# fevzibabaoglu/adaptive-edge-aware-jpeg

Measured on AMD Instinct MI355X. Metric: megapixels/sec encode (Canny+quadtree+DCT+quant), 4K batch, higher is better.
Workload: dtype f32; 1 GPU; 64 x 3840x2160 float32 RGB per GPU, YCbCr, blocks 4-64, quality 40-80 (BASELINE config 4: 512 4K images / 8 GPUs); images_per_gpu=64, height=2160, width=3840, color_space=YCbCr, steps_in_flight=4

## Files before the change

### adaptive_edge_aware_jpeg_amd/_lib.py

```python
import ctypes
import os
import threading

import numpy as np

_HERE = os.path.dirname(os.path.abspath(__file__))
LIB_PATH = os.environ.get("AEJ_LIBRARY") or os.path.join(_HERE, "libaejpeg_hip.so")

SPACE_IDS = {"YCbCr": 0, "YCoCg": 1, "YCoCg-R": 2, "OKLAB": 3, "ICtCp": 4, "ICaCb": 5, "JzAzBz": 6}
CONVERT_IDS = dict(SPACE_IDS, XYZ=7)

AEJ_ERR_ARG, AEJ_ERR_HIP, AEJ_ERR_STATE, AEJ_ERR_CAPACITY, AEJ_ERR_UNSUPPORTED = -1, -2, -3, -4, -5


class AejError(RuntimeError):
    pass


class AejPlan(ctypes.Structure):
    _fields_ = [
        ("batch", ctypes.c_int32), ("H", ctypes.c_int32), ("W", ctypes.c_int32),
        ("layer_h", ctypes.c_int32 * 3), ("layer_w", ctypes.c_int32 * 3), ("root_size", ctypes.c_int32 * 3),
        ("coeff_off", ctypes.c_int64 * 3), ("coeff_stride", ctypes.c_int64),
        ("leaf_off", ctypes.c_int64 * 3), ("leaf_stride", ctypes.c_int64),
        ("state_off", ctypes.c_int64 * 3), ("state_stride", ctypes.c_int64),
        ("workspace_bytes", ctypes.c_uint64),
    ]


_lib = None
_lib_lock = threading.Lock()

HIP_DEFAULT_HW_QUEUES = 4
_hw_queues = HIP_DEFAULT_HW_QUEUES
_hw_queues_source = "HIP default (assumed)"


def _look_at_hw_queues():
    global _hw_queues, _hw_queues_source
    present = os.environ.get("GPU_MAX_HW_QUEUES")
    if present is not None:
        try:
            v = int(present)
        except ValueError:
            v = 0
        if v > 0:
            _hw_queues, _hw_queues_source = v, "GPU_MAX_HW_QUEUES was in the environment when the package was imported"
    return _hw_queues


def configure_hw_queues(want=16):
    global _hw_queues, _hw_queues_source
    import sys
    if os.environ.get("GPU_MAX_HW_QUEUES") is not None:
        return _look_at_hw_queues()
    trusted = "torch" not in sys.modules
    os.environ["GPU_MAX_HW_QUEUES"] = str(int(want))
    if trusted:
        _hw_queues, _hw_queues_source = int(want), "configure_hw_queues() before torch was imported"
        for ctx in _contexts.values():
            ctx.check(ctx.lib.aej_set_hw_queues(ctx.handle, _hw_queues))
    return _hw_queues


def set_hw_queues(n):
    global _hw_queues, _hw_queues_source
    _hw_queues, _hw_queues_source = int(n), "stated by the application (set_hw_queues)"
    for ctx in _contexts.values():
        ctx.check(ctx.lib.aej_set_hw_queues(ctx.handle, _hw_queues))


def hw_queues():
    return _hw_queues, _hw_queues_source


_warned_queue_limited = False


def warn_if_queue_limited(ctx, batch, H, W):
    global _warned_queue_limited
    if _warned_queue_limited:
        return
    sch = ctx.schedule(batch, H, W)
    if sch["limited_by_hw_queues"]:
        _warned_queue_limited = True
        import warnings
        warnings.warn(f"adaptive_edge_aware_jpeg_amd: this call ({batch} x {W}x{H}) would run as more overlapping sub-batches with more hardware "
                      f"queues; the library schedules for {sch['hw_queues']} ({_hw_queues_source}).  Put GPU_MAX_HW_QUEUES=16 into the environment "
                      "(or call adaptive_edge_aware_jpeg_amd.configure_hw_queues()) before `import torch`, or state the runtime's real value with "
                      "set_hw_queues().", RuntimeWarning, stacklevel=3)


_P, _I, _I64, _U64 = ctypes.c_void_p, ctypes.c_int, ctypes.c_int64, ctypes.c_uint64
class CannyParams(ctypes.Structure):
    _fields_ = [("canny_low_ratio", ctypes.c_double), ("canny_high_ratio", ctypes.c_double), ("clahe_clip_limit", ctypes.c_double),
                ("bilateral_sigma_color", ctypes.c_double), ("bilateral_sigma_space", ctypes.c_double), ("use_l2_gradient", ctypes.c_int)]


class JpegDecHuff(ctypes.Structure):
    _fields_ = [("lut", ctypes.c_uint16 * 512), ("maxcode", ctypes.c_int32 * 18), ("valoff", ctypes.c_int32 * 18), ("vals", ctypes.c_uint8 * 256)]


class JpegDecDesc(ctypes.Structure):
    _fields_ = [("width", ctypes.c_int32), ("height", ctypes.c_int32), ("ncomp", ctypes.c_int32), ("hs", ctypes.c_int32), ("vs", ctypes.c_int32),
                ("mcux", ctypes.c_int32), ("mcuy", ctypes.c_int32), ("blocks_per_mcu", ctypes.c_int32), ("restart_interval", ctypes.c_int32),
                ("n_segments", ctypes.c_int32), ("sof", ctypes.c_int32), ("precision16", ctypes.c_int32),
                ("comp_id", ctypes.c_uint8 * 4), ("comp_h", ctypes.c_uint8 * 4), ("comp_v", ctypes.c_uint8 * 4), ("comp_tq", ctypes.c_uint8 * 4),
                ("qt", (ctypes.c_uint16 * 64) * 3), ("dc", JpegDecHuff * 3), ("ac", JpegDecHuff * 3),
                ("scan_offset", ctypes.c_int64), ("scan_length", ctypes.c_int64)]


class JpegProgFrame(ctypes.Structure):
    _fields_ = [("width", ctypes.c_int32), ("height", ctypes.c_int32), ("ncomp", ctypes.c_int32), ("hs", ctypes.c_int32), ("vs", ctypes.c_int32),
                ("mcux", ctypes.c_int32), ("mcuy", ctypes.c_int32), ("blocks_per_mcu", ctypes.c_int32), ("sof", ctypes.c_int32),
                ("precision16", ctypes.c_int32), ("n_scans", ctypes.c_int32), ("n_levels", ctypes.c_int32),
                ("comp_id", ctypes.c_uint8 * 4), ("comp_h", ctypes.c_uint8 * 4), ("comp_v", ctypes.c_uint8 * 4), ("comp_tq", ctypes.c_uint8 * 4),
                ("qt", (ctypes.c_uint16 * 64) * 3)]


class JpegProgScan(ctypes.Structure):
    _fields_ = [("ncomp", ctypes.c_int32), ("comp", ctypes.c_int32 * 4), ("td", ctypes.c_int32 * 4), ("ta", ctypes.c_int32 * 4),
                ("ss", ctypes.c_int32), ("se", ctypes.c_int32), ("ah", ctypes.c_int32), ("al", ctypes.c_int32),
                ("restart_interval", ctypes.c_int32), ("units_x", ctypes.c_int32), ("units_y", ctypes.c_int32),
                ("n_segments", ctypes.c_int32), ("level", ctypes.c_int32), ("dc", JpegDecHuff * 3), ("ac", JpegDecHuff),
                ("data_offset", ctypes.c_int64), ("data_length", ctypes.c_int64)]


SIGNATURES = {
    "aej_abi_version": (_I, []),
    "aej_create": (_P, [_I, _P]),
    "aej_destroy": (None, [_P]),
    "aej_last_error": (ctypes.c_char_p, [_P]),
    "aej_synchronize": (_I, [_P]),
    "aej_set_stream": (_I, [_P, _P]),
    "aej_get_hysteresis_stats": (_I, [_P, _P]),
    "aej_set_graph_mode": (_I, [_P, _I]),
    "aej_set_sub_batches": (_I, [_P, _I]),
    "aej_set_hw_queues": (_I, [_P, _I]),
    "aej_get_schedule_host": (_I, [_P, _I, _I, _I, _P]),
    "aej_set_option": (_I, [_P, ctypes.c_char_p, _I64]),
    "aej_get_option": (_I, [_P, ctypes.c_char_p, _P]),
    "aej_test_fail_after_stage": (_I, [_P, _I]),
    "aej_encode_batch_begin": (_I, [_P, _P, _I, _I, _I, _I, _P, _P, _P, _P, _P, _P, _U64]),
    "aej_encode_batch_end": (_I, [_P]),
    "aej_get_split_calls": (ctypes.c_int64, [_P]),
    "aej_get_graph_stats": (_I, [_P, _P]),
    "aej_set_profiling": (_I, [_P, _I]),
    "aej_get_stage_ms": (_I, [_P, _P]),
    "aej_stage_name": (ctypes.c_char_p, [_I]),
    "aej_set_settings": (_I, [_P, _I, _I, _I, _P]),
    "aej_encode_plan": (_I, [_P, _I, _I, _I, ctypes.POINTER(AejPlan)]),
    "aej_encode_batch": (_I, [_P, _P, _I, _I, _I, _P, _P, _P, _P, _P, _P, _U64]),
    "aej_encode_batch_u8": (_I, [_P, _P, _I, _I, _I, _P, _P, _P, _P, _P, _P, _U64]),
    "aej_metrics_workspace_bytes": (_U64, [_I, _I, _I]),
    "aej_metrics_batch": (_I, [_P, _P, _P, _I, _I, _I, _I, _P, _P, _U64]),
    "aej_color_convert": (_I, [_P, _I, _P, _P, _I64]),
    "aej_color_planes": (_I, [_P, _P, _I, _I, _I, _P, _P, _P]),
    "aej_canny_workspace_bytes": (_U64, [_I, _I]),
    "aej_canny": (_I, [_P, _P, _I, _I, _P, _P, _P, _P, _U64]),
    "aej_set_canny_params": (_I, [_P, _P]),
    "aej_quadtree_workspace_bytes": (_U64, [_I, _I, _I, _I]),
    "aej_quadtree_capacity": (_I, [_I, _I, _I, _I, ctypes.POINTER(_I64), ctypes.POINTER(_I64), ctypes.POINTER(_I64)]),
    "aej_quadtree": (_I, [_P, _P, _I, _I, _I, _I, _P, _P, _P, _P, _U64]),
    "aej_dct_quant_zigzag": (_I, [_P, _P, _I, _I, _I, _P, _I64, _P, _P]),
    "aej_deflate_stream_bound": (_U64, [_U64]),
    "aej_deflate_workspace_bytes": (_U64, [_P, _I, _I, _I]),
    "aej_deflate_histogram": (_I, [_P, _P, _P, _I, _I, _I, _P, _P, _U64]),
    "aej_deflate_batch": (_I, [_P, _P, _P, _I, _I, _I, _P, _I, _P, _U64, _P, _P, _U64]),
    "aej_deflate_build_tables": (_I, [_P, _P, _P]),
    "aej_pack_u8_levels_host": (_I, [_P, _I64, _P, _I]),
    "aej_decode_workspace_bytes": (_U64, [_P, _I, _I, _I]),
    "aej_decode_batch": (_I, [_P, _P, _P, _P, _I, _I, _I, _P, _P, _U64]),
    "aej_decode_batch_tables": (_I, [_P, _P, _P, _P, _I, _I, _I, _P, _P, _P, _U64]),
    "aej_requantise_batch": (_I, [_P, _P, _P, _P, _I, _I, _I, _I, _P, _P, _U64]),
    "aej_color_convert_inverse": (_I, [_P, _I, _P, _P, _I64]),
    "aej_leaf_positions_host": (_I64, [_P, _I64, _I, _I, _I, _P]),
    "aej_inflate_batch": (_I, [_P, _P, _P, _I, _P, _U64, _P, _P]),
    "aej_decode_headers_workspace_bytes": (_U64, [_P, _I, _I, _I]),
    "aej_decode_headers": (_I, [_P, _P, _P, _P, _I, _I, _I, _P, _P, _P, _P, _U64]),
    "aej_lpips_weights_bytes": (_U64, []),
    "aej_lpips_param_count": (_I64, []),
    "aej_lpips_pack_weights_host": (_I, [_P, _I64, _P]),
    "aej_lpips_features_bytes": (_U64, [_I, _I, _I]),
    "aej_lpips_workspace_bytes": (_U64, [_I, _I, _I]),
    "aej_lpips_features": (_I, [_P, _P, _P, _I, _I, _I, _P, _P, _U64]),
    "aej_lpips_batch": (_I, [_P, _P, _P, _P, _P, _I, _I, _I, _P, _P, _U64]),
    "aej_jfif_workspace_bytes": (_U64, [_I, _I, _I, _I]),
    "aej_jfif_headers_host": (_I, [_I, _I, _I, _P, _I]),
    "aej_jfif_encode_batch": (_I, [_P, _P, _I, _I, _I, _I, _P, _P, _U64, _P, _P, _P, _P, _U64]),
    "aej_jfif_recon_batch": (_I, [_P, _I, _I, _I, _I, _P, _P, _U64]),
    "aej_jfif_workspace_bytes_opt": (_U64, [_I, _I, _I, _I, _I, _I]),
    "aej_jfif_headers_host_opt": (_I, [_I, _I, _I, _I, _P, _I]),
    "aej_jfif_huffman_host": (_I, [_P, _P, _P, _I]),
    "aej_jfif_encode_batch_opt": (_I, [_P, _P, _I, _I, _I, _I, _P, _I, _I, _P, _U64, _P, _P, _P, _P, _U64]),
    "aej_jfif_recon_batch_opt": (_I, [_P, _I, _I, _I, _I, _I, _I, _P, _P, _U64]),
    "aej_jpegdec_parse_host": (_I, [_P, _U64, _P, _P, _I]),
    "aej_jpegdec_workspace_bytes": (_U64, [_P, _P, _I]),
    "aej_jpegdec_batch": (_I, [_P, _P, _I, _P, _U64, _P, _P, _U64, _P, _P, _P, _U64]),
    "aej_jpegdec_sync_rounds": (_I64, [_P]),
    "aej_jpegprog_parse_host": (_I, [_P, _U64, _P, _P, _I, _P, _I]),
    "aej_jpegprog_workspace_bytes": (_U64, [_P, _P, _P, _I]),
    "aej_jpegprog_batch": (_I, [_P, _P, _P, _I, _P, _U64, _P, _P, _U64, _P, _P, _P, _U64]),
    "aej_test_jpegprog_coefs": (_I, [_P, _P, _P, _I, _P, _U64, _P, _I, _P, _U64, _P, _P, _U64]),
    "aej_test_jpegprog_coefs_host": (_I, [_P, _P, _P, _U64, _I, _P, _U64]),
}

INFLATE_STATUS = ["ok", "bad zlib header", "bad block type", "bad code lengths", "invalid literal/length or distance code",
                  "distance too far back", "stored block LEN/NLEN mismatch", "truncated stream", "output over capacity",
                  "Adler-32 mismatch", "bad stream descriptor"]
JPEGDEC_STATUS = ["ok", "truncated scan (it ends before the last MCU)", "bad Huffman code", "coefficient run past 63",
                  "DC category above 11", "restart marker out of sequence, missing or unexpected"]
HEADER_STATUS = ["ok", "more leaves than the layer holds", "leaf size outside the block-size range of the header",
                 "quadtree header does not tile the layer", "coefficient count does not match the quadtree header", "bad layer descriptor"]


def load_library():
    global _lib
    with _lib_lock:
        if _lib is None:
            if not os.path.exists(LIB_PATH):
                raise AejError(
                    f"{LIB_PATH} is missing: build it with `python -c 'import __graft_entry__ as g; g.build()'` "
                    "(hipcc --offload-arch=gfx950).  There is no CPU fallback.")
            import torch
            lib = ctypes.CDLL(LIB_PATH)
            for name, (res, args) in SIGNATURES.items():
                fn = getattr(lib, name)
                fn.restype = res
                fn.argtypes = args
            _lib = lib
    return _lib


def _torch():
    import torch
    if not torch.cuda.is_available():
        raise AejError("no HIP device visible to PyTorch-ROCm: the adaptive-JPEG encode path runs on the GPU only")
    return torch


class Context:

    def __init__(self, device=0):
        self.torch = _torch()
        self.lib = load_library()
        self.device = self.torch.device("cuda", device if isinstance(device, int) else device.index or 0)
        self.stream = self.torch.cuda.current_stream(self.device).cuda_stream
        self.handle = self.lib.aej_create(self.device.index, ctypes.c_void_p(self.stream))
        if not self.handle:
            raise AejError(self.lib.aej_last_error(None).decode())
        self.check(self.lib.aej_set_hw_queues(self.handle, _hw_queues))
        self.settings_key = None
        self._ws = None

    def check_stream(self):
        cur = self.torch.cuda.current_stream(self.device).cuda_stream
        if cur != self.stream:
            raise AejError(f"context bound to stream {self.stream:#x} used while torch's current stream is {cur:#x}: "
                           "obtain the context with get_context() inside the `torch.cuda.stream(...)` block")

    def __del__(self):
        try:
            if getattr(self, "handle", None):
                self.lib.aej_destroy(self.handle)
                self.handle = None
        except Exception:
            pass

    def check(self, rc):
        if rc == 0:
            return
        msg = self.lib.aej_last_error(self.handle).decode()
        if rc == AEJ_ERR_ARG:
            raise ValueError(msg)
        if rc == AEJ_ERR_UNSUPPORTED:
            raise NotImplementedError(msg)
        raise AejError(f"aej error {rc}: {msg}")

    def empty(self, shape, dtype):
        return self.torch.empty(shape, dtype=dtype, device=self.device)

    def workspace(self, nbytes):
        self.check_stream()
        if self._ws is None or self._ws.numel() < nbytes:
            self._ws = None
            self._ws = self.torch.empty(int(nbytes), dtype=self.torch.uint8, device=self.device)
        return self._ws

    def pinned(self, nbytes):
        if getattr(self, "_pinned", None) is None or self._pinned.numel() < nbytes:
            self._pinned = None
            self._pinned = self.torch.empty(int(max(nbytes, 1 << 20)), dtype=self.torch.uint8, pin_memory=True)
        return self._pinned

    def hysteresis_stats(self):
        buf = (ctypes.c_int64 * 4)()
        self.check(self.lib.aej_get_hysteresis_stats(self.handle, ctypes.cast(buf, ctypes.c_void_p)))
        return {"calls": int(buf[0]), "queued": int(buf[1])}

    def set_canny_params(self, params=None):
        if params is None:
            self.check(self.lib.aej_set_canny_params(self.handle, None))
            return
        lo, hi, clip, sc, ss, l2 = params
        v = CannyParams(float(lo), float(hi), float(clip), float(sc), float(ss), 1 if l2 else 0)
        self.check(self.lib.aej_set_canny_params(self.handle, ctypes.cast(ctypes.pointer(v), ctypes.c_void_p)))

    def set_sub_batches(self, n):
        self.check(self.lib.aej_set_sub_batches(self.handle, int(n)))

    def schedule(self, batch, H, W):
        buf = (ctypes.c_int32 * 4)()
        self.check(self.lib.aej_get_schedule_host(self.handle, int(batch), int(H), int(W), ctypes.cast(buf, ctypes.c_void_p)))
        return {"hw_queues": int(buf[0]), "sub_batches": int(buf[1]), "limited_by_hw_queues": bool(buf[2]), "hw_queues_source": _hw_queues_source}

    def set_option(self, name, value):
        self.check(self.lib.aej_set_option(self.handle, name.encode(), int(value)))

    def get_option(self, name):
        v = ctypes.c_int64()
        self.check(self.lib.aej_get_option(self.handle, name.encode(), ctypes.cast(ctypes.pointer(v), ctypes.c_void_p)))
        return int(v.value)

    def split_calls(self):
        return int(self.lib.aej_get_split_calls(self.handle))

    def set_graph_mode(self, mode):
        self.check(self.lib.aej_set_graph_mode(self.handle, int(mode)))

    def graph_stats(self):
        buf = (ctypes.c_int64 * 3)()
        self.check(self.lib.aej_get_graph_stats(self.handle, ctypes.cast(buf, ctypes.c_void_p)))
        return {"launches": int(buf[0]), "captures": int(buf[1]), "cached": int(buf[2])}

    def to_device(self, arr, dtype):
        t = self.torch
        if isinstance(arr, t.Tensor):
            return arr.to(device=self.device, dtype=dtype).contiguous()
        return t.from_numpy(np.ascontiguousarray(arr)).to(device=self.device, dtype=dtype).contiguous()

    def set_settings(self, space, bmin, bmax, qmats):
        key = (space, bmin, bmax, qmats.tobytes())
        if key == self.settings_key:
            return
        q = np.ascontiguousarray(qmats, dtype=np.int32)
        self.check(self.lib.aej_set_settings(self.handle, SPACE_IDS[space], bmin, bmax, q.ctypes.data_as(ctypes.c_void_p)))
        self.settings_key = key

    N_STAGES = 18

    def set_profiling(self, on):
        self.check(self.lib.aej_set_profiling(self.handle, 1 if on else 0))

    def stage_ms(self):
        buf = (ctypes.c_float * self.N_STAGES)()
        self.check(self.lib.aej_get_stage_ms(self.handle, ctypes.cast(buf, ctypes.c_void_p)))
        return {self.lib.aej_stage_name(i).decode(): float(buf[i]) for i in range(self.N_STAGES)}

    def plan(self, batch, H, W):
        p = AejPlan()
        self.check(self.lib.aej_encode_plan(self.handle, batch, H, W, ctypes.byref(p)))
        return p


_contexts = {}


def get_context(device=0):
    idx = device if isinstance(device, int) else (device.index or 0)
    torch = _torch()
    key = (idx, torch.cuda.current_stream(torch.device("cuda", idx)).cuda_stream)
    ctx = _contexts.get(key)
    if ctx is None:
        ctx = _contexts[key] = Context(idx)
    return ctx


def release_context(ctx):
    for key, known in list(_contexts.items()):
        if known is ctx:
            del _contexts[key]
    ctx._ws = None
    ctx._pinned = None
    ctx._in_flight = None
    if getattr(ctx, "handle", None):
        ctx.lib.aej_destroy(ctx.handle)
        ctx.handle = None
```

### adaptive_edge_aware_jpeg_amd/csrc/aej_common.h

```cpp
#pragma once
#include <hip/hip_runtime.h>
#include <stdint.h>

namespace aej {

constexpr int kMaxSizes = 8;
constexpr int kClaheTiles = 4;
constexpr int kHystTile = 64;
constexpr int kBlurTW = 64, kBlurTH = 32;
constexpr int kQtChunk = 256;

struct Geom {
    int B;
    int nl;
    int H, W;
    int h[3], w[3];
    int rh[3], rw[3];
    long long poff[3];
    long long pstride;
    int tiled;
    int ctw[3], cth[3];
    int wpr[3];
    long long bpoff[3];
    long long bpstride;
};

struct QtGeom {
    int bmin, bmax;
    int cell;
    int root[3];
    int ncell[3];
    int ltot[3];
    long long pyr_off[3];
    long long pyr_stride;
    int nchunk[3];
    long long chunk_off[3];
    long long chunk_stride;
    long long coeff_off[3], coeff_stride;
    long long leaf_off[3], leaf_stride;
    long long state_off[3], state_stride;
    long long coeff_cap[3], leaf_cap[3], state_cap[3];
    int nsizes;
    long long work_off[3][kMaxSizes], work_stride[kMaxSizes];
};
struct Tuning {
    int color_strip = 1;
    int color_strip_rows = 0;
    int color_workgroups = 0;
    int planes_row_major = 0;
    int dct64_kernel = 0;
    int dct_small_workgroups = 0;
    int sobel_lds = 0;
    int dct_multi = 1;
    int sobel_xcd = 1;
};

constexpr int kChunkInts = 4 + kMaxSizes;
constexpr int kMaxPlanes = 3072;

constexpr int kMetricBand = 32;

struct LeafWork {
    unsigned xy;
    int coef;
};
__host__ __device__ __forceinline__ LeafWork pack_work(int x, int y, int coef)
{
    LeafWork w;
    w.xy = (unsigned)x | ((unsigned)y << 16);
    w.coef = coef;
    return w;
}
__device__ __forceinline__ int4 unpack_work(int plane, const LeafWork &w) { return make_int4(plane, (int)(w.xy & 0xffffu), (int)(w.xy >> 16), w.coef); }

struct DctTables {
    const float *D[kMaxSizes];
    const int *zzinv[kMaxSizes];
    const int *qm[3][kMaxSizes];
};

__host__ __device__ inline long long plane_elem(int tiled, int w, int y, int x)
{
    return tiled ? ((long long)(y >> 2) * (w >> 2) + (x >> 2)) * 16 + ((y & 3) << 2) + (x & 3) : (long long)y * w + x;
}

__host__ __device__ inline long long bp_index(int y, int xw, int wpr) { return ((long long)(y >> 6) * wpr + xw) * 64 + (y & 63); }
__host__ __device__ inline long long bp_words(int h, int wpr) { return (long long)((h + 63) / 64) * wpr * 64; }

inline int ilog2(int v) { int l = 0; while ((1 << l) < v) l++; return l; }

__device__ __forceinline__ int wave_scan_incl(int v)
{
    v += __builtin_amdgcn_update_dpp(0, v, 0x111, 0xf, 0xf, false);
    v += __builtin_amdgcn_update_dpp(0, v, 0x112, 0xf, 0xf, false);
    v += __builtin_amdgcn_update_dpp(0, v, 0x114, 0xf, 0xf, false);
    v += __builtin_amdgcn_update_dpp(0, v, 0x118, 0xf, 0xf, false);
    v += __builtin_amdgcn_update_dpp(0, v, 0x142, 0xa, 0xf, false);
    v += __builtin_amdgcn_update_dpp(0, v, 0x143, 0xc, 0xf, false);
    return v;
}
__device__ __forceinline__ unsigned wave_max_u32(unsigned v)
{
    auto mx = [](unsigned a, int b) { return a > (unsigned)b ? a : (unsigned)b; };
    v = mx(v, __builtin_amdgcn_update_dpp(0, (int)v, 0x111, 0xf, 0xf, false));
    v = mx(v, __builtin_amdgcn_update_dpp(0, (int)v, 0x112, 0xf, 0xf, false));
    v = mx(v, __builtin_amdgcn_update_dpp(0, (int)v, 0x114, 0xf, 0xf, false));
    v = mx(v, __builtin_amdgcn_update_dpp(0, (int)v, 0x118, 0xf, 0xf, false));
    v = mx(v, __builtin_amdgcn_update_dpp(0, (int)v, 0x142, 0xa, 0xf, false));
    v = mx(v, __builtin_amdgcn_update_dpp(0, (int)v, 0x143, 0xc, 0xf, false));
    return (unsigned)__builtin_amdgcn_readlane((int)v, 63);
}
__device__ __forceinline__ int wave_total(int v) { return __builtin_amdgcn_readlane(wave_scan_incl(v), 63); }

}

#define AEJ_HIP_CHECK(expr)                                                       \
    do {                                                                          \
        hipError_t _e = (expr);                                                   \
        if (_e != hipSuccess) return aej::hip_fail(ctx, _e, #expr, __FILE__, __LINE__); \
    } while (0)
```

### adaptive_edge_aware_jpeg_amd/csrc/aej_launch.h

```cpp
#pragma once
#include "aej_common.h"

namespace aej {

int launch_color_convert(hipStream_t st, int space, const float *rgb, float *out, long long n);
bool color_planes_can_tile(const Geom &g, int space, bool in_u8, const Tuning &t);
int launch_color_planes(hipStream_t st, int space, const void *rgb, bool in_u8, const Geom &g, const float *mid, const float *scale,
                        float *raw, float *norm, unsigned char *u8, int *tile_hist, const Tuning &t);
struct AreaTabs {
    int mode;
    int isx, isy;
    const int *xoff, *xsi, *yoff, *ysi;
    const float *xal, *yal;
};
int launch_color_planes_generic(hipStream_t st, int space, const void *rgb, bool in_u8, const Geom &g, const float *mid, const float *scale,
                                const AreaTabs &tabs, float *raw, float *norm, unsigned char *u8, int *tile_hist);
void launch_plane_u8(hipStream_t st, const float *plane, const Geom &g, unsigned char *u8, int *tile_hist);

struct CannyBuffers {
    unsigned char *u8a;
    unsigned char *u8b;
    int *tile_hist;
    unsigned char *lut;
    int *blur_hist;
    int *thr;
    unsigned long long *weak;
    unsigned long long *strong;
    int *hflags;
    int *hlist;
    int *pass_count;
    const float *space_w;
    const float *color_w;
    double low_q = 0.10 * 100, high_q = 0.30 * 100;
    double clip_limit = 0.75;
    int l2 = 1;
    unsigned char *dump_clahe, *dump_gauss;
};
constexpr int kHystCounters = 128;
long long hyst_tiles_per_image(const Geom &g);
int hyst_ring_slots(const Geom &g);
void launch_clahe_pad_hist(hipStream_t st, const Geom &g, const CannyBuffers &cb);
void launch_clahe_lut(hipStream_t st, const Geom &g, const CannyBuffers &cb);
void launch_clahe_blur(hipStream_t st, const Geom &g, const CannyBuffers &cb);
void launch_thresholds(hipStream_t st, const Geom &g, const CannyBuffers &cb);
void launch_sobel_nms(hipStream_t st, const Geom &g, const CannyBuffers &cb, const Tuning &t);
void launch_hysteresis(hipStream_t st, const Geom &g, const CannyBuffers &cb);
void launch_zero(hipStream_t st, void *p16, size_t bytes_multiple_of_16);
void launch_bits_to_edge(hipStream_t st, const Geom &g, const unsigned long long *strong, unsigned char *edge01);
void launch_bits_to_map(hipStream_t st, const Geom &g, const unsigned long long *weak, const unsigned long long *strong, unsigned char *map);

struct QtBuffers {
    unsigned char *pyr;
    const unsigned long long *edge_bits;
    int *chunk_cnt;
    unsigned short *lane_code;
    int *leaves;
    unsigned char *states;
    long long *counts;
    LeafWork *work[kMaxSizes];
    int *work_count;
    long long work_cap[kMaxSizes];
    int *overflow;
};
void launch_qt_cells(hipStream_t st, const Geom &g, const QtGeom &q, const unsigned long long *edge_bits, const QtBuffers &qb);
void launch_pack_edge_bits(hipStream_t st, const Geom &g, const unsigned char *edge, unsigned long long *bits);
void launch_qt_count(hipStream_t st, const Geom &g, const QtGeom &q, const QtBuffers &qb);
void launch_qt_scan(hipStream_t st, const Geom &g, const QtGeom &q, const QtBuffers &qb);
void launch_qt_emit(hipStream_t st, const Geom &g, const QtGeom &q, const QtBuffers &qb);

constexpr int kBigBlocks = 128;
constexpr int kMaxBlock = 1024;
constexpr int big_blocks(int S) { return S <= 256 ? kBigBlocks : S == 512 ? 64 : 32; }
constexpr long long big_scratch_floats_for(int S) { return S >= 256 ? (long long)big_blocks(S) * S * S : 0; }
struct DctArgs {
    const float *norm;
    int *coeffs;
    float *dct_f32;
    const LeafWork *work;
    float *scratch;
    const int *work_count;
    int k;
    int nplanes;
    const float *D;
    const int *zzinv;
    const int *qm[3];
    int crowded = 0;
};
int launch_dct(hipStream_t st, int size, const Geom &g, const QtGeom &q, const DctArgs &a, long long max_items, const Tuning &t);
int launch_dct_multi(hipStream_t st, const Geom &g, const QtGeom &q, const DctArgs *args, const long long *max_items);
void launch_work_from_leaves(hipStream_t st, const int *leaves, long long n, int bmin, int plane, LeafWork *const *work, int *work_count);


struct IdctArgs {
    const int *coeffs;
    float *planes;
    const LeafWork *work;
    float *scratch;
    const int *work_count;
    int k, nplanes;
    const float *D;
    const int *zz, *zzinv;
    const int *qm[3];
    float mid[3], scale[3];
};
void launch_work_from_tables(hipStream_t st, const Geom &g, const QtGeom &q, const int *leaves, const long long *counts, LeafWork *const *work,
                             int *work_count, int *bad );
int launch_idct(hipStream_t st, int size, const Geom &g, const QtGeom &q, const IdctArgs &a, long long max_items);
int launch_color_inverse(hipStream_t st, int space, const float *in, float *out, long long n);
int launch_upsample_color(hipStream_t st, int space, const Geom &g, const float *planes, float *rgb);

unsigned long long deflate_stream_bound(unsigned long long raw_bytes);
unsigned long long deflate_workspace_bytes(int batch, const long long *coeff_cap );
void launch_deflate_parse(hipStream_t st, const int *coeffs, const long long *counts, int batch, long long coeff_stride, const long long *coeff_off,
                          const long long *coeff_cap, int *hist, void *workspace);
void launch_deflate(hipStream_t st, const int *coeffs, const long long *counts, int batch, long long coeff_stride, const long long *coeff_off,
                    const long long *coeff_cap, const unsigned *tables , int reuse_parse, unsigned char *out,
                    unsigned long long stream_stride, long long *sizes, void *workspace);

void launch_inflate(hipStream_t st, const unsigned char *src, const long long *desc, int n, unsigned char *dst, long long dst_bytes,
                    long long *out_bytes, int *status);

struct HdrGeom {
    int bmin, bmax;
    int h[3], w[3];
    int proot[3];
    long long leaf_off[3], leaf_span[3], leaf_stride;
    long long coeff_span[3];
};
void launch_headers(hipStream_t st, const unsigned char *states, const long long *desc, const long long *inflated, int nlayers, const HdrGeom &g,
                    unsigned char *codes, int *leaves, long long *counts, int *status);

void launch_requant_check(hipStream_t st, const Geom &g, const QtGeom &q, const int *leaves, const long long *counts, const int *qmats,
                          long long qmat_words, int *bad);
int launch_requant(hipStream_t st, const Geom &g, const QtGeom &q, const float *dct, const int *leaves, const long long *counts, int n_sets,
                   const int *qmats, const int *const *zz, int *out, long long set_stride, int *bad, int blocks_per_plane);

struct MetricParts {
    long long stride;
    int psnr_n;
    long long grey_off, grey_n;
    long long lvl_off[5], lvl_n[5];
};
int metric_prep_blocks(long long npx);
long long ssim_partials(int h, int w);
void launch_metric_prep(hipStream_t st, const float *a, const float *b, int B, long long npx, double *part, long long stride, unsigned char *ga,
                        unsigned char *gb);
void launch_metric_pool_grey(hipStream_t st, const unsigned char *ga, const unsigned char *gb, int B, int H, int W, int f, int hp, int wp, float *xa,
                             float *xb);
void launch_ssim_level(hipStream_t st, bool interleaved, const float *xa, const float *xb, int B, int C, int h, int w, const float *g11, double *part,
                       long long stride, long long off, bool want_ss, float *pool_a = nullptr, float *pool_b = nullptr);
void launch_pool2_rgb(hipStream_t st, const float *ia, const float *ib, int B, int h, int w, int p, int h2, int w2, float *oa, float *ob);
void launch_pool2(hipStream_t st, bool interleaved, const float *in, int B, int C, int h, int w, int p, int h2, int w2, float *out);
void launch_metric_final(hipStream_t st, const double *part, const MetricParts &P, int B, long long npx, long long n_ssim, const long long *n_level, double *out);


constexpr int kLpipsTaps = 5;
constexpr int kLpipsHeadPixels = 256;
struct LpipsLayer { int cin, cinp, cout, k, stride, pad; };
extern const LpipsLayer kLpipsLayers[kLpipsTaps];
struct LpipsGeom {
    int H, W;
    int h[kLpipsTaps], w[kLpipsTaps];
    int ph[2], pw[2];
    long long tap_off[kLpipsTaps];
    long long feat_elems;
    long long x_elems, y_elems;
    int nblk[kLpipsTaps], max_blk;
};
bool lpips_geom(int H, int W, LpipsGeom &g);
long long lpips_param_floats();
long long lpips_packed_floats(long long off[kLpipsTaps][3]);
void lpips_pack_host(const float *params, float *packed);
void launch_lpips(hipStream_t st, const float *wpk, const float *img, int B, const LpipsGeom &g, float *X, float *Y, float *feats_out,
                  const float *feats_a, double *partial, double *out);


constexpr int kJfifBlockWords = 52;
constexpr int kJfifBlockWordsOpt = 53;
constexpr int kJfifHdrMax = 1024;
struct JfifGeom {
    int B, H, W, nq;
    int mcux, mcuy, ybx, yby;
    int yw, yh, cw, ch;
    long long n_mcu, nblk;
    long long stream_words, n_chunks;
    long long plane_bytes;
    int hs, vs, opt, pad_;
};
struct JfifParams {
    int qt[2][64];
    int hdr_len, dht_off, pad_[2];
    unsigned char hdr[kJfifHdrMax];
};
struct JfifBufs {
    JfifParams *par; int *dct; short *coef; int *lens; long long *boff, *btot; unsigned *stream; int *ffcnt; long long *ffpre, *fftot, *total;
    unsigned char *planes;
    unsigned long long *hist; unsigned *codes; unsigned char *fhdr; int *fhdr_len;
};
bool jfif_geom(int B, int H, int W, int nq, JfifGeom &g, int ss = 2, int opt = 0);
unsigned long long jfif_carve(void *base, const JfifGeom &g, JfifBufs &w);
void jfif_quant_tables(int q, int luma[64], int chroma[64]);
void jfif_params_host(int q, int H, int W, JfifParams &p, int ss = 2);
int jfif_huffman_host(const long long *counts, unsigned char *bits, unsigned char *huffval);
hipError_t launch_jfif_encode(hipStream_t st, const JfifGeom &g, const JfifBufs &w, const JfifParams *par_host, const unsigned char *rgb,
                              unsigned char *out, unsigned long long cap, long long *lengths, long long *offsets);
hipError_t launch_jfif_recon(hipStream_t st, const JfifGeom &g, const JfifBufs &w, unsigned char *rgb_out);

}

#include <string>
#include <vector>
#include "jpegdec_core.h"

namespace aej {
struct JdBufSizes { long long chunks, segs, slots, blocks, clean, planes, px; };
struct JdBufs {
    JdFile *files; aej_jpegdec_desc *descs; int *last_change;
    int *cnt; long long *pre, *clean_len; JdSeg *segs; unsigned char *clean; JdSlots sl; short *coef; unsigned char *planes;
};
struct JdHuffSrc { bool defined = false; unsigned char bits[17] = {}; unsigned char vals[256] = {}; int count = 0; };
bool jd_build_huff(const JdHuffSrc &s, aej_jpegdec_huff &h);
int jpegdec_parse(const unsigned char *data, unsigned long long n, aej_jpegdec_desc &d, std::string &msg);
long long jpegdec_layout(const aej_jpegdec_desc *descs, int n, int S, std::vector<JdFile> &files, JdBufSizes &z);
unsigned long long jpegdec_carve(void *base, int n, const JdBufSizes &z, JdBufs &w);
hipError_t launch_jpegdec_begin(hipStream_t st, int n, const JdBufSizes &z, const JdBufs &w, const void *blob_host, unsigned long long blob_bytes,
                                const unsigned char *scans, int S, int *status);
hipError_t launch_jpegdec_unstuff(hipStream_t st, int n, const JdBufSizes &z, const JdBufs &w, const unsigned char *scans, int S, int *status);
hipError_t launch_jpegdec_recon(hipStream_t st, int n, const JdBufSizes &z, const JdBufs &w, unsigned char *out);
hipError_t launch_jpegdec_sync(hipStream_t st, int n, const JdBufSizes &z, const JdBufs &w, int S, int first_round, int rounds);
hipError_t launch_jpegdec_finish(hipStream_t st, int n, const JdBufSizes &z, const JdBufs &w, int S, unsigned char *out, int *status);

}

#include "jpegprog_core.h"

namespace aej {
struct JpLayout {
    std::vector<JdFile> sfiles, ffiles;
    std::vector<aej_jpegdec_desc> sdescs, fdescs;
    std::vector<JpScan> scans;
    std::vector<int> src;
    std::vector<JpItem> items;
    std::vector<long long> level_items;
    JdBufSizes sz{}, fz{};
    int n_levels = 0;
};
struct JpBufs { void *blob; JdBufs s, f; JpScan *scans; JpItem *items; int *sstatus; };
int jpegprog_parse(const unsigned char *data, unsigned long long n, aej_jpegprog_frame &f, std::vector<aej_jpegprog_scan> &scans, std::string &msg);
bool jpegprog_layout(const aej_jpegprog_frame *frames, const aej_jpegprog_scan *scans, int n, JpLayout &y);
unsigned long long jpegprog_blob(const JpLayout &y, std::vector<unsigned char> *out);
unsigned long long jpegprog_carve(void *base, const JpLayout &y, JpBufs &w);
hipError_t launch_jpegprog_entropy(hipStream_t st, const JpLayout &y, const JpBufs &w, const void *blob_host, unsigned long long blob_bytes,
                                   const unsigned char *data, int n_levels, int *status);
hipError_t launch_jpegprog_recon(hipStream_t st, const JpLayout &y, const JpBufs &w, unsigned char *out);
int jpegprog_coefs_host(const aej_jpegprog_frame &frame, const aej_jpegprog_scan *scans, const unsigned char *file, unsigned long long nbytes,
                        int n_levels, short *coef, unsigned long long coef_blocks);

}
```

### adaptive_edge_aware_jpeg_amd/csrc/api.hip

```cpp
#include <math.h>
#include <stdarg.h>
#include <stdio.h>
#include <stdlib.h>
#include <string.h>

#include <algorithm>
#include <atomic>
#include <string>
#include <thread>
#include <vector>

#include "../../include/aej.h"
#include "../../include/aej_testing.h"
#include "aej_common.h"
#include "aej_launch.h"

using namespace aej;

struct aej_pending;
constexpr int kFlagWords = 16;
struct aej_ctx {
    int device = 0;
    hipStream_t stream = nullptr;
    std::string err;
    bool has_settings = false;
    int space = 0, bmin = 0, bmax = 0, nsizes = 0;
    void *tables = nullptr;
    const float *d_D[kMaxSizes] = {};
    const int *d_zzinv[kMaxSizes] = {};
    const int *d_zz[kMaxSizes] = {};
    const int *d_qm[3][kMaxSizes] = {};
    int *d_check = nullptr;
    const float *d_space_w = nullptr, *d_color_w = nullptr;
    float *d_bilateral = nullptr;
    aej_canny_params canny = { 0.10, 0.30, 0.75, 75.0, 75.0, 1 };
    int *h_flag = nullptr;
    long long last_hyst_queued = 0;
    bool capturing = false;
    long long n_encode_calls = 0;
    int graph_mode = 0;
    hipStream_t gstream = nullptr;
    hipEvent_t gevent = nullptr;
    struct GraphEntry {
        const void *rgb; void *coeffs, *leaves, *states, *counts, *dct, *ws;
        int batch, H, W, in_u8;
        hipGraphExec_t exec;
        unsigned long long last_use;
    };
    std::vector<GraphEntry> graphs;
    unsigned long long graph_clock = 0, n_graph_launches = 0, n_graph_captures = 0;
    int sub_mode = 0;
    int hw_queues = 4;
    int fail_after = -1;
    static constexpr int kMaxSub = 8;
    int dct_crowded = 0;
    hipStream_t sub_stream[kMaxSub] = {};
    hipEvent_t sub_color_done[kMaxSub] = {}, sub_in = nullptr;
    int *sub_flag[kMaxSub] = {};
    long long n_split_calls = 0;
    int sub_chain = -1;
    int chain_hook = 0;
    hipEvent_t chain_event = nullptr;
    Tuning tune;
    int jd_subseq_bits = 2048;
    long long jd_sync_rounds = 0;
    struct aej_pending *pending = nullptr;
    bool profiling = false;
    hipEvent_t ev[24] = {};
    int ev_stage[24] = {};
    int n_ev = 0;
    float stage_ms[AEJ_N_STAGES] = {};
};

namespace aej {
static int fail(aej_ctx *ctx, int code, const char *fmt, ...)
{
    char buf[512];
    va_list ap;
    va_start(ap, fmt);
    vsnprintf(buf, sizeof buf, fmt, ap);
    va_end(ap);
    if (ctx) ctx->err = buf;
    return code;
}
int hip_fail(aej_ctx *ctx, hipError_t e, const char *expr, const char *file, int line)
{
    return fail(ctx, AEJ_ERR_HIP, "%s failed: %s (%s:%d)", expr, hipGetErrorString(e), file, line);
}
}

static void mark(aej_ctx *ctx, int stage)
{
    if (!ctx->profiling || ctx->n_ev >= 24) return;
    if (!ctx->ev[ctx->n_ev] && hipEventCreate(&ctx->ev[ctx->n_ev]) != hipSuccess) return;
    ctx->ev_stage[ctx->n_ev] = stage;
    (void)hipEventRecord(ctx->ev[ctx->n_ev], ctx->stream);
    ctx->n_ev++;
}

extern "C" const char *aej_stage_name(int i);
static int injected_failure(aej_ctx *ctx, int stage)
{
    if (ctx->fail_after != stage) return 0;
    ctx->fail_after = -1;
    ctx->err = std::string("injected failure after stage ") + aej_stage_name(stage);
    return AEJ_ERR_STATE;
}

static void collect_marks(aej_ctx *ctx)
{
    for (int i = 0; i < AEJ_N_STAGES; i++) ctx->stage_ms[i] = 0.f;
    for (int i = 1; i < ctx->n_ev; i++) {
        float ms = 0.f;
        if (hipEventElapsedTime(&ms, ctx->ev[i - 1], ctx->ev[i]) == hipSuccess && ctx->ev_stage[i] >= 0) ctx->stage_ms[ctx->ev_stage[i]] += ms;
    }
}

#include <mutex>
static std::mutex g_chain_mutex;
constexpr int kMaxDevices = 64;
static hipEvent_t g_last_color_done[kMaxDevices] = {};
static int g_calls_in_flight[kMaxDevices] = {};

static void free_pending(aej_ctx *ctx);
static bool call_in_flight(const aej_ctx *ctx);

static void drop_graphs(aej_ctx *ctx)
{
    for (auto &e : ctx->graphs) if (e.exec) (void)hipGraphExecDestroy(e.exec);
    ctx->graphs.clear();
}

static const int kRatios[7][3][2] = {
    { { 1, 1 }, { 2, 2 }, { 2, 2 } },
    { { 1, 1 }, { 2, 2 }, { 2, 2 } },
    { { 1, 1 }, { 2, 2 }, { 2, 2 } },
    { { 1, 1 }, { 2, 2 }, { 2, 2 } },
    { { 1, 1 }, { 1, 4 }, { 1, 4 } },
    { { 1, 1 }, { 1, 4 }, { 1, 4 } },
    { { 1, 1 }, { 2, 2 }, { 2, 2 } },
};
static const double kMid[7][3] = {
    { 0.5000000037252903, 7.450580596923828e-09, 0.0 }, { 0.5, 0.0, 0.0 }, { 0.5, 0.0, 0.0 },
    { 0.4999999, 0.021152213, -0.056563325 }, { 0.07497266, -0.0008235276, 0.023989676 },
    { 0.07498085, 0.02180194, -0.018250957 }, { 0.0087900255, 0.00048353244, -0.0020741792 },
};
static const double kScale[7][3] = {
    { 253.99999810755253, 254.000003784895, 254.0 }, { 254.0, 254.0, 254.0 }, { 254.0, 127.0, 127.0 },
    { 254.00005, 497.9055, 497.94604 }, { 1693.9674, 1133.9044, 1694.004 },
    { 1693.7823, 1838.5665, 1330.3855 }, { 14448.194, 7590.505, 5552.201 },
};

static bool is_pow2(int v) { return v > 0 && (v & (v - 1)) == 0; }
static long long align_up(long long v, long long a) { return (v + a - 1) / a * a; }

static int root_size_of(int h, int w)
{
    int n = h > w ? h : w;
    int lp;
    if (n <= 2) lp = n;
    else { lp = 1; while (lp * 2 < n) lp *= 2; }
    return lp * 2;
}

static void fill_clahe_geom(Geom &g)
{
    long long bp = 0;
    for (int l = 0; l < g.nl; l++) {
        g.wpr[l] = (g.w[l] + 63) / 64;
        g.bpoff[l] = bp;
        bp += bp_words(g.h[l], g.wpr[l]);
    }
    g.bpstride = bp;
    for (int l = 0; l < g.nl; l++) {
        int w = g.w[l], h = g.h[l];
        int wp = w, hp = h;
        if ((w % 4) != 0 || (h % 4) != 0) { wp = w + (4 - w % 4); hp = h + (4 - h % 4); }
        g.ctw[l] = wp / 4;
        g.cth[l] = hp / 4;
    }
}

static int make_geom(aej_ctx *ctx, int space, int B, int H, int W, Geom &g)
{
    memset(&g, 0, sizeof g);
    if (H > 65535 || W > 65535) return fail(ctx, AEJ_ERR_UNSUPPORTED, "image %dx%d: sides above 65535 pixels are not built (leaf origins travel as 16-bit pairs, LeafWork)", H, W);
    g.B = B; g.nl = 3; g.H = H; g.W = W;
    long long off = 0;
    for (int l = 0; l < 3; l++) {
        g.rh[l] = kRatios[space][l][0];
        g.rw[l] = kRatios[space][l][1];
        g.h[l] = H / g.rh[l];
        g.w[l] = W / g.rw[l];
        if (g.h[l] < 1 || g.w[l] < 1) return fail(ctx, AEJ_ERR_ARG, "image %dx%d too small for the down-sampling ratios", H, W);
        g.poff[l] = off;
        off += align_up((long long)g.h[l] * g.w[l], 64);
    }
    g.pstride = off;
    fill_clahe_geom(g);
    return 0;
}

static void make_plane_geom(int H, int W, Geom &g)
{
    memset(&g, 0, sizeof g);
    g.B = 1; g.nl = 1; g.H = H; g.W = W;
    g.h[0] = H; g.w[0] = W; g.rh[0] = g.rw[0] = 1;
    g.poff[0] = 0;
    g.pstride = align_up((long long)H * W, 64);
    fill_clahe_geom(g);
}

static int make_qtgeom(aej_ctx *ctx, const Geom &g, int bmin, int bmax, QtGeom &q, bool allow_small_root = false)
{
    memset(&q, 0, sizeof q);
    if (!is_pow2(bmin) || !is_pow2(bmax) || bmin > bmax || bmin < 1)
        return fail(ctx, AEJ_ERR_ARG, "block sizes must be powers of two with min <= max (got %d, %d)", bmin, bmax);
    q.bmin = bmin; q.bmax = bmax; q.cell = bmin;
    long long pyr = 0, chunks = 0, co = 0, lo = 0, so = 0;
    for (int l = 0; l < g.nl; l++) {
        int root = root_size_of(g.h[l], g.w[l]);
        if (root < bmin) {
            if (!allow_small_root || g.nl != 1) return fail(ctx, AEJ_ERR_UNSUPPORTED, "layer %d (%dx%d): root %d smaller than min block %d", l, g.h[l], g.w[l], root, bmin);
            q.cell = root;
        }
        q.root[l] = root;
        q.ncell[l] = root / q.cell;
        q.ltot[l] = ilog2(q.ncell[l]);
        if (q.ltot[l] > 14) return fail(ctx, AEJ_ERR_UNSUPPORTED, "quadtree deeper than 14 levels");
        q.pyr_off[l] = pyr;
        long long states = 0;
        for (int j = 0; j <= q.ltot[l]; j++) { long long s = q.ncell[l] >> j; states += s * s; }
        pyr += align_up(states, 256);
        long long nc2 = (long long)q.ncell[l] * q.ncell[l];
        q.nchunk[l] = (int)(nc2 / 256 > 0 ? nc2 / 256 : 1);
        q.chunk_off[l] = chunks;
        chunks += q.nchunk[l];
        int top = bmax < root ? bmax : root;
        long long wc = align_up(g.w[l], top), hc = align_up(g.h[l], top);
        if (wc > root) wc = root;
        if (hc > root) hc = root;
        q.coeff_cap[l] = wc * hc;
        q.leaf_cap[l] = (wc / q.cell) * (hc / q.cell);
        q.state_cap[l] = states;
        q.coeff_off[l] = co; co += align_up(q.coeff_cap[l], 64);
        q.leaf_off[l] = lo;  lo += align_up(q.leaf_cap[l], 16);
        q.state_off[l] = so; so += align_up(q.state_cap[l], 64);
    }
    q.pyr_stride = pyr; q.chunk_stride = chunks;
    q.coeff_stride = co; q.leaf_stride = lo; q.state_stride = so;
    int k = 0;
    for (int s = bmin; s <= bmax && k < kMaxSizes; s *= 2, k++) {
        long long off = 0;
        for (int l = 0; l < g.nl; l++) {
            q.work_off[l][k] = off;
            if (s > q.root[l]) continue;
            int top = bmax < q.root[l] ? bmax : q.root[l];
            long long wc = align_up(g.w[l], top), hc = align_up(g.h[l], top);
            if (wc > q.root[l]) wc = q.root[l];
            if (hc > q.root[l]) hc = q.root[l];
            off += ((wc + s - 1) / s) * ((hc + s - 1) / s);
        }
        q.work_stride[k] = off;
    }
    q.nsizes = k;
    return 0;
}

struct Carver {
    char *base;
    unsigned long long off = 0;
    explicit Carver(void *p) : base(static_cast<char *>(p)) {}
    template <typename T> T *take(long long n)
    {
        off = (off + 255) & ~255ull;
        T *p = base ? reinterpret_cast<T *>(base + off) : nullptr;
        off += (unsigned long long)n * sizeof(T);
        return p;
    }
};

struct CannyWs {
    CannyBuffers cb;
    char *zero_begin, *zero_end;
};

static void carve_canny(Carver &c, const Geom &g, CannyWs &w)
{
    memset(&w, 0, sizeof w);
    long long planes = (long long)g.B * g.pstride;
    long long tiles = hyst_tiles_per_image(g) * g.B;
    w.cb.u8a = c.take<unsigned char>(planes);
    w.cb.u8b = c.take<unsigned char>(planes);
    w.cb.weak = c.take<unsigned long long>((long long)g.B * g.bpstride);
    w.cb.strong = c.take<unsigned long long>((long long)g.B * g.bpstride);
    w.cb.lut = c.take<unsigned char>((long long)g.B * 3 * 16 * 256);
    w.cb.thr = c.take<int>((long long)g.B * 3 * 2);
    w.zero_begin = reinterpret_cast<char *>(c.take<int>(0));
    w.cb.hlist = c.take<int>(hyst_ring_slots(g));
    w.cb.tile_hist = c.take<int>((long long)g.B * 3 * 16 * 256);
    w.cb.blur_hist = c.take<int>((long long)g.B * 3 * 256);
    w.cb.pass_count = c.take<int>(kHystCounters);
    w.cb.hflags = c.take<int>(2 * tiles);
    c.take<int>(0);
    w.zero_end = c.base ? c.base + c.off : nullptr;
}

struct QtWs {
    QtBuffers qb;
    char *zero_begin, *zero_end;
};

static void carve_qt(Carver &c, const Geom &g, const QtGeom &q, bool with_work, QtWs &w)
{
    memset(&w, 0, sizeof w);
    w.zero_begin = reinterpret_cast<char *>(c.take<int>(0));
    w.qb.pyr = c.take<unsigned char>((long long)g.B * q.pyr_stride);
    w.qb.overflow = c.take<int>(1);
    c.take<int>(0);
    w.zero_end = c.base ? c.base + c.off : nullptr;
    w.qb.chunk_cnt = c.take<int>((long long)g.B * q.chunk_stride * kChunkInts);
    w.qb.lane_code = c.take<unsigned short>((long long)g.B * q.chunk_stride * 64);
    if (with_work) {
        w.qb.work_count = c.take<int>((long long)g.B * 3 * kMaxSizes);
        for (int k = 0; k < q.nsizes; k++) {
            long long cap = q.work_stride[k] * g.B;
            w.qb.work_cap[k] = cap;
            w.qb.work[k] = c.take<LeafWork>(cap > 0 ? cap : 1);
        }
    } else {
        w.qb.work_count = nullptr;
    }
}

extern "C" int aej_abi_version(void) { return AEJ_ABI_VERSION; }

extern "C" aej_ctx *aej_create(int device, void *hip_stream)
{
    int n = 0;
    if (hipGetDeviceCount(&n) != hipSuccess || device < 0 || device >= n || device >= kMaxDevices) return nullptr;
    if (hipSetDevice(device) != hipSuccess) return nullptr;
    aej_ctx *ctx = new aej_ctx();
    ctx->device = device;
    ctx->stream = static_cast<hipStream_t>(hip_stream);
    if (hipHostMalloc(reinterpret_cast<void **>(&ctx->h_flag), kFlagWords * sizeof(int), hipHostMallocDefault) != hipSuccess) { delete ctx; return nullptr; }
    return ctx;
}

extern "C" void aej_destroy(aej_ctx *ctx)
{
    if (!ctx) return;
    (void)hipSetDevice(ctx->device);
    if (call_in_flight(ctx)) {
        (void)hipDeviceSynchronize();
        std::lock_guard<std::mutex> lock(g_chain_mutex);
        if (g_calls_in_flight[ctx->device] > 0) g_calls_in_flight[ctx->device]--;
    }
    free_pending(ctx);
    {
        std::lock_guard<std::mutex> lock(g_chain_mutex);
        for (int i = 0; i < aej_ctx::kMaxSub; i++)
            if (ctx->sub_color_done[i] && g_last_color_done[ctx->device] == ctx->sub_color_done[i]) g_last_color_done[ctx->device] = nullptr;
    }
    drop_graphs(ctx);
    if (ctx->gstream) (void)hipStreamDestroy(ctx->gstream);
    if (ctx->gevent) (void)hipEventDestroy(ctx->gevent);
    if (ctx->tables) (void)hipFree(ctx->tables);
    if (ctx->d_bilateral) (void)hipFree(ctx->d_bilateral);
    for (int i = 0; i < aej_ctx::kMaxSub; i++) {
        if (ctx->sub_stream[i]) (void)hipStreamDestroy(ctx->sub_stream[i]);
        if (ctx->sub_color_done[i]) (void)hipEventDestroy(ctx->sub_color_done[i]);
        if (ctx->sub_flag[i]) (void)hipHostFree(ctx->sub_flag[i]);
    }
    if (ctx->sub_in) (void)hipEventDestroy(ctx->sub_in);
    if (ctx->h_flag) (void)hipHostFree(ctx->h_flag);
    for (int i = 0; i < 24; i++) if (ctx->ev[i]) (void)hipEventDestroy(ctx->ev[i]);
    delete ctx;
}

extern "C" const char *aej_last_error(aej_ctx *ctx)
{
    if (!ctx) return "aej: no context (aej_create failed: no such HIP device?)";
    return ctx->err.c_str();
}

extern "C" int aej_synchronize(aej_ctx *ctx)
{
    if (!ctx) return AEJ_ERR_ARG;
    if (call_in_flight(ctx)) return fail(ctx, AEJ_ERR_STATE, "%s between aej_encode_batch_begin and aej_encode_batch_end", __func__);
    AEJ_HIP_CHECK(hipStreamSynchronize(ctx->stream));
    return 0;
}

static void zigzag_order(int s, std::vector<int> &zz)
{
    zz.resize((size_t)s * s);
    int i = 0;
    for (int d = 0; d < 2 * s - 1; d++) {
        int lo = d - s + 1 > 0 ? d - s + 1 : 0, hi = d < s - 1 ? d : s - 1;
        if (d % 2) for (int r = lo; r <= hi; r++) zz[i++] = r * s + (d - r);
        else for (int r = hi; r >= lo; r--) zz[i++] = r * s + (d - r);
    }
}

extern "C" int aej_set_settings(aej_ctx *ctx, int space, int bmin, int bmax, const int32_t *qmats_host)
{
    if (!ctx) return AEJ_ERR_ARG;
    if (call_in_flight(ctx)) return fail(ctx, AEJ_ERR_STATE, "aej_set_settings between aej_encode_batch_begin and aej_encode_batch_end");
    if (space < 0 || space > 6) return fail(ctx, AEJ_ERR_ARG, "Unsupported color space id: %d", space);
    if (!is_pow2(bmin) || !is_pow2(bmax) || bmin > bmax || bmin < 2)
        return fail(ctx, AEJ_ERR_ARG, "block size range (%d, %d): powers of two with 2 <= min <= max required", bmin, bmax);
    if (bmax > kMaxBlock)
        return fail(ctx, AEJ_ERR_UNSUPPORTED, "block size range (%d, %d): no kernel for blocks above %d", bmin, bmax, kMaxBlock);
    if (ilog2(bmax) - ilog2(bmin) + 1 > kMaxSizes)
        return fail(ctx, AEJ_ERR_UNSUPPORTED, "block size range (%d, %d) spans more than %d sizes", bmin, bmax, kMaxSizes);
    if (!qmats_host) return fail(ctx, AEJ_ERR_ARG, "qmats_host is NULL");
    AEJ_HIP_CHECK(hipSetDevice(ctx->device));
    int nsizes = 0;
    for (int s = bmin; s <= bmax; s *= 2) nsizes++;
    std::vector<char> blob;
    auto put = [&](const void *p, size_t bytes) {
        size_t o = (blob.size() + 255) & ~(size_t)255;
        blob.resize(o + bytes);
        memcpy(blob.data() + o, p, bytes);
        return o;
    };
    size_t oD[kMaxSizes], oZ[kMaxSizes], oZf[kMaxSizes], oQ[3][kMaxSizes];
    int k = 0;
    size_t qpos = 0;
    std::vector<size_t> qoff_layer_size;
    for (int s = bmin; s <= bmax; s *= 2, k++) {
        std::vector<float> D((size_t)s * s);
        for (int u = 0; u < s; u++) {
            double alpha = u == 0 ? sqrt(1.0 / (double)s) : sqrt(2.0 / (double)s);
            for (int n = 0; n < s; n++) D[(size_t)u * s + n] = (float)(alpha * cos(3.14159265358979323846 * (double)(2 * n + 1) * (double)u / (2.0 * (double)s)));
        }
        oD[k] = put(D.data(), D.size() * 4);
        std::vector<int> zz, inv((size_t)s * s);
        zigzag_order(s, zz);
        for (int i = 0; i < s * s; i++) inv[zz[i]] = i;
        oZ[k] = put(inv.data(), inv.size() * 4);
        oZf[k] = put(zz.data(), zz.size() * 4);
    }
    for (int l = 0; l < 3; l++) {
        k = 0;
        for (int s = bmin; s <= bmax; s *= 2, k++) {
            for (int i = 0; i < s * s; i++)
                if (qmats_host[qpos + i] < 1) return fail(ctx, AEJ_ERR_ARG, "quantisation matrix entries must be >= 1");
            oQ[l][k] = put(qmats_host + qpos, (size_t)s * s * 4);
            qpos += (size_t)s * s;
        }
    }
    const int zero_words[64] = {};
    const size_t oCheck = put(zero_words, sizeof zero_words);
    drop_graphs(ctx);
    if (ctx->tables) { AEJ_HIP_CHECK(hipStreamSynchronize(ctx->stream)); AEJ_HIP_CHECK(hipFree(ctx->tables)); ctx->tables = nullptr; }
    AEJ_HIP_CHECK(hipMalloc(&ctx->tables, blob.size()));
    AEJ_HIP_CHECK(hipMemcpy(ctx->tables, blob.data(), blob.size(), hipMemcpyHostToDevice));
    char *base = static_cast<char *>(ctx->tables);
    for (int i = 0; i < kMaxSizes; i++) {
        ctx->d_D[i] = nullptr; ctx->d_zzinv[i] = nullptr; ctx->d_zz[i] = nullptr;
        for (int l = 0; l < 3; l++) ctx->d_qm[l][i] = nullptr;
    }
    for (int i = 0; i < nsizes; i++) {
        ctx->d_D[i] = reinterpret_cast<const float *>(base + oD[i]);
        ctx->d_zzinv[i] = reinterpret_cast<const int *>(base + oZ[i]);
        ctx->d_zz[i] = reinterpret_cast<const int *>(base + oZf[i]);
        for (int l = 0; l < 3; l++) ctx->d_qm[l][i] = reinterpret_cast<const int *>(base + oQ[l][i]);
    }
    ctx->d_check = reinterpret_cast<int *>(base + oCheck);
    ctx->space = space; ctx->bmin = bmin; ctx->bmax = bmax; ctx->nsizes = nsizes;
    ctx->has_settings = true;
    return 0;
}

static int ensure_canny_tables(aej_ctx *ctx)
{
    if (ctx->d_color_w) return 0;
    float tab[16 + 256] = { 0 };
    double sigc = ctx->canny.bilateral_sigma_color, sigs = ctx->canny.bilateral_sigma_space;
    if (sigc <= 0) sigc = 1;
    if (sigs <= 0) sigs = 1;
    const double cc = -0.5 / (sigc * sigc), sc = -0.5 / (sigs * sigs);
    for (int i = 0; i < 256; i++) tab[16 + i] = (float)exp((double)i * (double)i * cc);
    int t = 0;
    for (int i = -2; i <= 2; i++)
        for (int j = -2; j <= 2; j++) {
            double r = sqrt((double)i * i + (double)j * j);
            if (r > 2.0) continue;
            tab[t++] = (float)exp(r * r * sc);
        }
    if (!ctx->d_bilateral) AEJ_HIP_CHECK(hipMalloc(&ctx->d_bilateral, sizeof tab));
    AEJ_HIP_CHECK(hipStreamSynchronize(ctx->stream));
    AEJ_HIP_CHECK(hipMemcpy(ctx->d_bilateral, tab, sizeof tab, hipMemcpyHostToDevice));
    ctx->d_space_w = ctx->d_bilateral;
    ctx->d_color_w = ctx->d_bilateral + 16;
    return 0;
}

static void apply_canny_params(const aej_ctx *ctx, CannyBuffers &cb)
{
    cb.space_w = ctx->d_space_w;
    cb.color_w = ctx->d_color_w;
    cb.low_q = ctx->canny.canny_low_ratio * 100;
    cb.high_q = ctx->canny.canny_high_ratio * 100;
    cb.clip_limit = ctx->canny.clahe_clip_limit;
    cb.l2 = ctx->canny.use_l2_gradient ? 1 : 0;
}

extern "C" int aej_set_canny_params(aej_ctx *ctx, const aej_canny_params *p)
{
    if (!ctx) return AEJ_ERR_ARG;
    if (call_in_flight(ctx)) return fail(ctx, AEJ_ERR_STATE, "aej_set_canny_params between aej_encode_batch_begin and aej_encode_batch_end");
    const aej_canny_params def = { 0.10, 0.30, 0.75, 75.0, 75.0, 1 };
    const aej_canny_params v = p ? *p : def;
    if (!(v.canny_low_ratio >= 0.0 && v.canny_low_ratio <= 1.0 && v.canny_high_ratio >= 0.0 && v.canny_high_ratio <= 1.0))
        return fail(ctx, AEJ_ERR_ARG, "Canny threshold ratios must lie in [0, 1] (np.percentile takes 0..100)");
    if (!(v.clahe_clip_limit == v.clahe_clip_limit) || !(v.bilateral_sigma_color == v.bilateral_sigma_color) || !(v.bilateral_sigma_space == v.bilateral_sigma_space))
        return fail(ctx, AEJ_ERR_ARG, "NaN Canny hyper-parameter");
    const bool tables_change = v.bilateral_sigma_color != ctx->canny.bilateral_sigma_color || v.bilateral_sigma_space != ctx->canny.bilateral_sigma_space;
    ctx->canny = v;
    drop_graphs(ctx);
    if (tables_change) { ctx->d_color_w = nullptr; ctx->d_space_w = nullptr; }
    return 0;
}

static int run_canny_chain(aej_ctx *ctx, const Geom &g, CannyWs &w)
{
    hipStream_t st = ctx->stream;
    launch_clahe_pad_hist(st, g, w.cb);
    launch_clahe_lut(st, g, w.cb);
    mark(ctx, AEJ_STAGE_CLAHE_LUT);
    auto publish = [&]() {
        std::lock_guard<std::mutex> lock(g_chain_mutex);
        if (hipEventRecord(ctx->chain_event, st) == hipSuccess) g_last_color_done[ctx->device] = ctx->chain_event;
    };
    launch_clahe_blur(st, g, w.cb);
    mark(ctx, AEJ_STAGE_CLAHE_BLUR);
    if (ctx->chain_hook == 2) publish();
    launch_thresholds(st, g, w.cb);
    mark(ctx, AEJ_STAGE_THRESHOLDS);
    launch_sobel_nms(st, g, w.cb, ctx->tune);
    mark(ctx, AEJ_STAGE_SOBEL_NMS);
    if (ctx->chain_hook == 3) publish();
    launch_hysteresis(st, g, w.cb);
    mark(ctx, AEJ_STAGE_HYSTERESIS);
    AEJ_HIP_CHECK(hipGetLastError());
    return 0;
}

static int clear_canny_ws(aej_ctx *ctx, const CannyWs &w)
{
    if (ctx->capturing) launch_zero(ctx->stream, w.zero_begin, (size_t)(w.zero_end - w.zero_begin));
    else AEJ_HIP_CHECK(hipMemsetAsync(w.zero_begin, 0, (size_t)(w.zero_end - w.zero_begin), ctx->stream));
    return 0;
}

static int run_quadtree(aej_ctx *ctx, const Geom &g, const QtGeom &q, QtWs &w, const unsigned long long *edge_bits)
{
    hipStream_t st = ctx->stream;
    if (ctx->capturing) launch_zero(st, w.zero_begin, (size_t)(w.zero_end - w.zero_begin));
    else AEJ_HIP_CHECK(hipMemsetAsync(w.zero_begin, 0, (size_t)(w.zero_end - w.zero_begin), st));
    w.qb.edge_bits = edge_bits;
    launch_qt_cells(st, g, q, edge_bits, w.qb);
    launch_qt_count(st, g, q, w.qb);
    launch_qt_scan(st, g, q, w.qb);
    launch_qt_emit(st, g, q, w.qb);
    AEJ_HIP_CHECK(hipGetLastError());
    return 0;
}

static void area_tab(int ssize, int dsize, double scale, std::vector<int> &off, std::vector<int> &si, std::vector<float> &alpha)
{
    off.assign((size_t)dsize + 1, 0); si.clear(); alpha.clear();
    for (int dx = 0; dx < dsize; dx++) {
        double fsx1 = dx * scale, fsx2 = fsx1 + scale;
        double cell = scale < ssize - fsx1 ? scale : ssize - fsx1;
        int sx1 = (int)ceil(fsx1), sx2 = (int)floor(fsx2);
        if (sx2 > ssize - 1) sx2 = ssize - 1;
        if (sx1 > sx2) sx1 = sx2;
        off[dx] = (int)si.size();
        if (sx1 - fsx1 > 1e-3) { si.push_back(sx1 - 1); alpha.push_back((float)((sx1 - fsx1) / cell)); }
        for (int sx = sx1; sx < sx2; sx++) { si.push_back(sx); alpha.push_back((float)(1.0 / cell)); }
        if (fsx2 - sx2 > 1e-3) {
            double a = fsx2 - sx2;
            if (a > 1.) a = 1.;
            if (a > cell) a = cell;
            si.push_back(sx2); alpha.push_back((float)(a / cell));
        }
    }
    off[dsize] = (int)si.size();
}

static long long area_tab_ints(const Geom &g)
{
    return 2LL * (g.w[1] + 1 + g.h[1] + 1) + 2LL * (g.W + 2 * g.w[1] + 2) + 2LL * (g.H + 2 * g.h[1] + 2) + 64;
}

static bool planes_fast_ok(const Geom &g)
{
    bool ok = (g.W % 4) == 0 && (g.H % 2) == 0;
    for (int l = 1; l < 3; l++) ok = ok && g.h[l] * g.rh[l] == g.H && g.w[l] * g.rw[l] == g.W;
    return ok;
}

static int run_color_planes(aej_ctx *ctx, const void *rgb, bool in_u8, const Geom &g, float *raw, float *norm, unsigned char *u8, int *hist,
                            int *tab_ws)
{
    float mid[3], scale[3];
    for (int i = 0; i < 3; i++) { mid[i] = (float)kMid[ctx->space][i]; scale[i] = (float)kScale[ctx->space][i]; }
    if (planes_fast_ok(g)) {
        Tuning t = ctx->tune;
        if (t.color_workgroups == 0 && ctx->dct_crowded && ctx->space < 3) t.color_workgroups = 224;
        if (launch_color_planes(ctx->stream, ctx->space, rgb, in_u8, g, mid, scale, raw, norm, u8, hist, t)) return fail(ctx, AEJ_ERR_ARG, "bad colour space");
        return 0;
    }
    AreaTabs t;
    memset(&t, 0, sizeof t);
    double sx = 1.0 / ((double)g.w[1] / (double)g.W), sy = 1.0 / ((double)g.h[1] / (double)g.H);
    int isx = (int)lrint(sx), isy = (int)lrint(sy);
    bool fast = fabs(sx - isx) < 2.220446049250313e-16 && fabs(sy - isy) < 2.220446049250313e-16;
    t.isx = isx; t.isy = isy;
    if (fast) t.mode = (isx == 2 && isy == 2) ? 0 : 1;
    else {
        t.mode = 2;
        if (!tab_ws) return fail(ctx, AEJ_ERR_STATE, "no workspace for the INTER_AREA tables");
        std::vector<int> xoff, xsi, yoff, ysi;
        std::vector<float> xal, yal;
        area_tab(g.W, g.w[1], sx, xoff, xsi, xal);
        area_tab(g.H, g.h[1], sy, yoff, ysi, yal);
        std::vector<int> blob;
        auto put_i = [&](const std::vector<int> &v) { size_t o = blob.size(); blob.insert(blob.end(), v.begin(), v.end()); return o; };
        auto put_f = [&](const std::vector<float> &v) { size_t o = blob.size(); blob.resize(o + v.size()); memcpy(blob.data() + o, v.data(), v.size() * 4); return o; };
        size_t o1 = put_i(xoff), o2 = put_i(xsi), o3 = put_f(xal), o4 = put_i(yoff), o5 = put_i(ysi), o6 = put_f(yal);
        if ((long long)blob.size() > area_tab_ints(g)) return fail(ctx, AEJ_ERR_CAPACITY, "INTER_AREA tables larger than reserved");
        AEJ_HIP_CHECK(hipMemcpyAsync(tab_ws, blob.data(), blob.size() * 4, hipMemcpyHostToDevice, ctx->stream));
        AEJ_HIP_CHECK(hipStreamSynchronize(ctx->stream));
        t.xoff = tab_ws + o1; t.xsi = tab_ws + o2; t.xal = reinterpret_cast<const float *>(tab_ws + o3);
        t.yoff = tab_ws + o4; t.ysi = tab_ws + o5; t.yal = reinterpret_cast<const float *>(tab_ws + o6);
    }
    if (launch_color_planes_generic(ctx->stream, ctx->space, rgb, in_u8, g, mid, scale, t, raw, norm, u8, hist)) return fail(ctx, AEJ_ERR_ARG, "bad colour space");
    return 0;
}

static long long big_scratch_floats(int bmax)
{
    long long m = 0;
    for (int s = 256; s <= bmax; s *= 2) m = std::max(m, big_scratch_floats_for(s));
    return m;
}

struct EncodeWs {
    float *big;
    float *norm;
    int *area_tabs;
    CannyWs canny;
    QtWs qt;
    unsigned long long bytes;
};

static void carve_encode(void *base, const Geom &g, const QtGeom &q, EncodeWs &w)
{
    Carver c(base);
    w.norm = c.take<float>((long long)g.B * g.pstride);
    w.area_tabs = c.take<int>(area_tab_ints(g));
    carve_canny(c, g, w.canny);
    carve_qt(c, g, q, true, w.qt);
    w.big = big_scratch_floats(q.bmax) ? c.take<float>(big_scratch_floats(q.bmax)) : nullptr;
    w.bytes = (c.off + 255) & ~255ull;
}

static unsigned long long sub_ws_bytes(Geom g, const QtGeom &q, int nsub);

static int check_encode_args(aej_ctx *ctx, int batch, int H, int W)
{
    if (!ctx) return AEJ_ERR_ARG;
    if (!ctx->has_settings) return fail(ctx, AEJ_ERR_STATE, "aej_set_settings has not been called");
    if (batch < 1 || H < 1 || W < 1) return fail(ctx, AEJ_ERR_ARG, "batch, H, W must be positive");
    if (batch * 3 > kMaxPlanes) return fail(ctx, AEJ_ERR_UNSUPPORTED, "batch %d too large for one call (max %d images)", batch, kMaxPlanes / 3);
    return 0;
}

extern "C" int aej_encode_plan(aej_ctx *ctx, int batch, int H, int W, aej_plan *plan)
{
    int rc = check_encode_args(ctx, batch, H, W);
    if (rc) return rc;
    if (!plan) return fail(ctx, AEJ_ERR_ARG, "plan is NULL");
    Geom g;
    QtGeom q;
    if ((rc = make_geom(ctx, ctx->space, batch, H, W, g))) return rc;
    if ((rc = make_qtgeom(ctx, g, ctx->bmin, ctx->bmax, q))) return rc;
    EncodeWs w;
    carve_encode(nullptr, g, q, w);
    memset(plan, 0, sizeof *plan);
    plan->batch = batch; plan->H = H; plan->W = W;
    for (int l = 0; l < 3; l++) {
        plan->layer_h[l] = g.h[l]; plan->layer_w[l] = g.w[l]; plan->root_size[l] = q.root[l];
        plan->coeff_off[l] = q.coeff_off[l]; plan->leaf_off[l] = q.leaf_off[l]; plan->state_off[l] = q.state_off[l];
    }
    plan->coeff_stride = q.coeff_stride; plan->leaf_stride = q.leaf_stride; plan->state_stride = q.state_stride;
    plan->workspace_bytes = w.bytes;
    for (int n = 2; n <= aej_ctx::kMaxSub && n <= batch; n++)
        plan->workspace_bytes = std::max<uint64_t>(plan->workspace_bytes, sub_ws_bytes(g, q, n) * (unsigned long long)n);
    return 0;
}

constexpr long long kGraphAutoPixels = 8LL << 20;

static int enqueue_back(aej_ctx *ctx, const Geom &g, const QtGeom &q, EncodeWs &w, int32_t *coeffs, float *dct_f32)
{
    hipStream_t st = ctx->stream;
    int rc;
    if ((rc = run_quadtree(ctx, g, q, w.qt, w.canny.cb.strong))) return rc;
    mark(ctx, AEJ_STAGE_QUADTREE);
    DctArgs args[kMaxSizes];
    int k = 0;
    for (int s = q.bmin; s <= q.bmax; s *= 2, k++) {
        DctArgs &a = args[k];
        a.norm = w.norm; a.coeffs = coeffs; a.dct_f32 = dct_f32;
        a.work = w.qt.qb.work[k]; a.work_count = w.qt.qb.work_count; a.k = k; a.nplanes = g.B * 3;
        a.scratch = w.big;
        a.D = ctx->d_D[k]; a.zzinv = ctx->d_zzinv[k];
        a.crowded = ctx->dct_crowded;
        for (int l = 0; l < 3; l++) a.qm[l] = ctx->d_qm[l][k];
    }
    const bool one_launch = ctx->tune.dct_multi && !ctx->profiling && (long long)g.B * g.H * g.W <= kGraphAutoPixels;
    if (!(one_launch && launch_dct_multi(st, g, q, args, w.qt.qb.work_cap) == 0)) {
        k = 0;
        for (int s = q.bmin; s <= q.bmax; s *= 2, k++) {
            if (launch_dct(st, s, g, q, args[k], w.qt.qb.work_cap[k], ctx->tune)) return fail(ctx, AEJ_ERR_UNSUPPORTED, "no DCT kernel for block size %d with %d planes", s, args[k].nplanes);
            mark(ctx, AEJ_STAGE_DCT_2 + ilog2(s) - 1);
        }
    }
    AEJ_HIP_CHECK(hipGetLastError());
    return 0;
}

static int enqueue_readback(aej_ctx *ctx, EncodeWs &w)
{
    AEJ_HIP_CHECK(hipMemcpyAsync(ctx->h_flag, w.qt.qb.overflow, sizeof(int), hipMemcpyDeviceToHost, ctx->stream));
    AEJ_HIP_CHECK(hipMemcpyAsync(ctx->h_flag + 1, w.canny.cb.pass_count + 32 , sizeof(int), hipMemcpyDeviceToHost, ctx->stream));
    return 0;
}

constexpr size_t kMaxGraphs = 8;

static int encode_graph(aej_ctx *ctx, const void *rgb, bool in_u8, const Geom &g, const QtGeom &q, EncodeWs &w, int32_t *coeffs, int32_t *leaves,
                        uint8_t *states, int64_t *counts, float *dct_f32, void *workspace, bool &used)
{
    used = false;
    if (!ctx->gstream) {
        AEJ_HIP_CHECK(hipStreamCreateWithFlags(&ctx->gstream, hipStreamNonBlocking));
        AEJ_HIP_CHECK(hipEventCreateWithFlags(&ctx->gevent, hipEventDisableTiming));
    }
    aej_ctx::GraphEntry *hit = nullptr;
    for (auto &e : ctx->graphs)
        if (e.rgb == rgb && e.coeffs == coeffs && e.leaves == leaves && e.states == states && e.counts == counts && e.dct == dct_f32 && e.ws == workspace &&
            e.batch == g.B && e.H == g.H && e.W == g.W && e.in_u8 == (int)in_u8) { hit = &e; break; }
    hipStream_t user = ctx->stream;
    if (!hit) {
        if (ctx->graphs.size() >= kMaxGraphs) {
            size_t lru = 0;
            for (size_t i = 1; i < ctx->graphs.size(); i++) if (ctx->graphs[i].last_use < ctx->graphs[lru].last_use) lru = i;
            if (ctx->graphs[lru].exec) (void)hipGraphExecDestroy(ctx->graphs[lru].exec);
            ctx->graphs.erase(ctx->graphs.begin() + (long)lru);
        }
        ctx->graphs.push_back({ rgb, coeffs, leaves, states, counts, dct_f32, workspace, g.B, g.H, g.W, (int)in_u8, nullptr, ++ctx->graph_clock });
        return 0;
    }
    if (!hit->exec) {
        hipGraph_t graph = nullptr;
        ctx->stream = ctx->gstream;
        ctx->capturing = true;
        hipError_t e = hipStreamBeginCapture(ctx->gstream, hipStreamCaptureModeThreadLocal);
        int rc = e == hipSuccess ? 0 : hip_fail(ctx, e, "hipStreamBeginCapture", __FILE__, __LINE__);
        if (!rc) rc = clear_canny_ws(ctx, w.canny);
        if (!rc) rc = run_color_planes(ctx, rgb, in_u8, g, nullptr, w.norm, w.canny.cb.u8a, w.canny.cb.tile_hist, w.area_tabs);
        if (!rc) {
            hipStream_t st = ctx->stream;
            launch_clahe_pad_hist(st, g, w.canny.cb);
            launch_clahe_lut(st, g, w.canny.cb);
            launch_clahe_blur(st, g, w.canny.cb);
            launch_thresholds(st, g, w.canny.cb);
            launch_sobel_nms(st, g, w.canny.cb, ctx->tune);
            launch_hysteresis(st, g, w.canny.cb);
            rc = enqueue_back(ctx, g, q, w, coeffs, dct_f32);
        }
        hipError_t e2 = e == hipSuccess ? hipStreamEndCapture(ctx->gstream, &graph) : hipSuccess;
        ctx->stream = user;
        ctx->capturing = false;
        if (rc || e2 != hipSuccess || !graph) {
            if (graph) (void)hipGraphDestroy(graph);
            (void)hipGetLastError();
            return rc ? rc : 0;
        }
        hipGraphExec_t exec = nullptr;
        e = hipGraphInstantiate(&exec, graph, nullptr, nullptr, 0);
        (void)hipGraphDestroy(graph);
        if (e != hipSuccess || !exec) { (void)hipGetLastError(); return 0; }
        hit->exec = exec;
        ctx->n_graph_captures++;
    }
    hit->last_use = ++ctx->graph_clock;
    AEJ_HIP_CHECK(hipEventRecord(ctx->gevent, user));
    AEJ_HIP_CHECK(hipStreamWaitEvent(ctx->gstream, ctx->gevent, 0));
    AEJ_HIP_CHECK(hipGraphLaunch(hit->exec, ctx->gstream));
    ctx->stream = ctx->gstream;
    const int rb = enqueue_readback(ctx, w);
    ctx->stream = user;
    if (rb) return rb;
    AEJ_HIP_CHECK(hipStreamSynchronize(ctx->gstream));
    ctx->n_graph_launches++;
    used = true;
    return 0;
}

static int sub_batches(const aej_ctx *ctx, const Geom &g, int hw_queues, bool as_if_unprofiled = false)
{
    if (ctx->sub_mode == 1 || (ctx->profiling && !as_if_unprofiled) || ctx->graph_mode == 2 || !planes_fast_ok(g)) return 1;
    int n = ctx->sub_mode;
    if (n == 0) {
        const long long px = (long long)g.B * g.H * g.W;
        if (hw_queues >= 8) {
            n = (px >= (384LL << 20) && g.B >= 16) ? 4 : (px >= (64LL << 20) && g.B >= 8) ? 2 : 1;
        } else {
            bool alone;
            { std::lock_guard<std::mutex> lock(g_chain_mutex); alone = g_calls_in_flight[ctx->device] == 0; }
            n = (alone && px >= (64LL << 20) && g.B >= 8) ? 2 : 1;
        }
    }
    if (n > aej_ctx::kMaxSub) n = aej_ctx::kMaxSub;
    if (n > g.B) n = g.B;
    return n;
}

static unsigned long long encode_ws_bytes(const Geom &g, const QtGeom &q)
{
    EncodeWs w;
    carve_encode(nullptr, g, q, w);
    return w.bytes;
}

static unsigned long long sub_ws_bytes(Geom g, const QtGeom &q, int nsub)
{
    g.B = (g.B + nsub - 1) / nsub;
    return encode_ws_bytes(g, q);
}

struct EncodePart { Geom g; EncodeWs w; bool whole_call = false; int32_t *coeffs = nullptr; float *dct = nullptr; hipStream_t stream = nullptr; int *flag = nullptr; bool used = false; };
struct aej_pending {
    bool active = false, complete = false;
    QtGeom q;
    std::vector<EncodePart> parts;
};

static void free_pending(aej_ctx *ctx) { delete ctx->pending; ctx->pending = nullptr; }

static bool call_in_flight(const aej_ctx *ctx) { return ctx->pending && ctx->pending->active; }

static aej_pending &pending_of(aej_ctx *ctx)
{
    if (!ctx->pending) ctx->pending = new aej_pending;
    return *ctx->pending;
}

static int enqueue_part(aej_ctx *ctx, EncodePart &p, const QtGeom &q, const void *rgb, bool in_u8, hipEvent_t done)
{
    int rc;
    mark(ctx, -1);
    if ((rc = clear_canny_ws(ctx, p.w.canny))) return rc;
// ... 571 lines not shown
    if (rc) return rc;
    if (call_in_flight(ctx)) return fail(ctx, AEJ_ERR_STATE, "%s between aej_encode_batch_begin and aej_encode_batch_end", __func__);
    if (!dct_f32 || !leaves || !counts || !qmats_dev || !coeffs_out) return fail(ctx, AEJ_ERR_ARG, "NULL buffer");
    if (n_sets < 1) return fail(ctx, AEJ_ERR_ARG, "n_sets must be at least 1 (got %d)", n_sets);
    AEJ_HIP_CHECK(hipSetDevice(ctx->device));
    Geom g;
    QtGeom q;
    if ((rc = make_geom(ctx, ctx->space, batch, H, W, g))) return rc;
    if ((rc = make_qtgeom(ctx, g, ctx->bmin, ctx->bmax, q))) return rc;
    const unsigned long long need = (unsigned long long)batch * q.coeff_stride;
    if (n_sets > 1 && set_stride_elems < need)
        return fail(ctx, AEJ_ERR_ARG, "set_stride_elems %llu is smaller than the batch's coefficients (%llu)", (unsigned long long)set_stride_elems, need);
    long long lw = 0;
    for (int s = ctx->bmin; s <= ctx->bmax; s *= 2) lw += (long long)s * s;
    long long maxcap = 0;
    for (int l = 0; l < 3; l++) maxcap = std::max(maxcap, q.coeff_cap[l]);
    const int blocks = (int)std::min<long long>(512, std::max<long long>(1, (maxcap + 16383) / 16384));
    hipStream_t st = ctx->stream;
    AEJ_HIP_CHECK(hipMemsetAsync(ctx->d_check, 0, sizeof(int), st));
    launch_requant_check(st, g, q, leaves, reinterpret_cast<const long long *>(counts), qmats_dev, (long long)n_sets * 3 * lw, ctx->d_check);
    launch_requant(st, g, q, dct_f32, leaves, reinterpret_cast<const long long *>(counts), n_sets, qmats_dev, ctx->d_zz, coeffs_out,
                   (long long)set_stride_elems, ctx->d_check, blocks);
    AEJ_HIP_CHECK(hipGetLastError());
    AEJ_HIP_CHECK(hipMemcpyAsync(ctx->h_flag, ctx->d_check, sizeof(int), hipMemcpyDeviceToHost, st));
    AEJ_HIP_CHECK(hipStreamSynchronize(st));
    if (*ctx->h_flag == 2) return fail(ctx, AEJ_ERR_ARG, "quantisation matrix entries must be >= 1");
    if (*ctx->h_flag) return fail(ctx, AEJ_ERR_ARG, "the leaf tables do not fit the plan (leaf count, block size outside %d-%d, origin or coefficient offset outside the layer)", q.bmin, q.bmax);
    return 0;
}

static int deflate_geometry(aej_ctx *ctx, int batch, int H, int W, QtGeom &q)
{
    int rc = check_encode_args(ctx, batch, H, W);
    if (rc) return rc;
    Geom g;
    if ((rc = make_geom(ctx, ctx->space, batch, H, W, g))) return rc;
    return make_qtgeom(ctx, g, ctx->bmin, ctx->bmax, q);
}

extern "C" uint64_t aej_deflate_stream_bound(uint64_t raw_bytes) { return deflate_stream_bound(raw_bytes); }

namespace aej { int deflate_build_table_host(const int *hist , int cover_all, unsigned *table ); }
extern "C" int aej_deflate_build_tables(const int32_t *hist_host, const int32_t *cover_all, uint32_t *tables_host)
{
    if (!hist_host || !tables_host) return AEJ_ERR_ARG;
    for (int l = 0; l < 3; l++)
        if (deflate_build_table_host(hist_host + l * AEJ_DEFLATE_HIST_BINS, cover_all ? cover_all[l] : 1, tables_host + l * AEJ_DEFLATE_TABLE_WORDS)) return AEJ_ERR_CAPACITY;
    return 0;
}

extern "C" int aej_pack_u8_levels_host(const float *rgb_host, int64_t n, uint8_t *u8_host, int threads)
{
    if (!rgb_host || !u8_host || n < 0) return AEJ_ERR_ARG;
    float lut[256];
    for (int k = 0; k < 256; k++) lut[k] = (float)k / 255.0f;
    const int64_t kBlock = 1 << 16;
    const int64_t nblocks = (n + kBlock - 1) / kBlock;
    int nt = threads < 1 ? 1 : threads > 64 ? 64 : threads;
    if ((int64_t)nt > nblocks) nt = nblocks > 0 ? (int)nblocks : 1;
    std::atomic<int64_t> next(0);
    std::atomic<int> exact(1);
    auto work = [&]() {
        for (;;) {
            const int64_t blk = next.fetch_add(1);
            if (blk >= nblocks || !exact.load(std::memory_order_relaxed)) return;
            const int64_t lo = blk * kBlock, hi = std::min(n, lo + kBlock);
            unsigned bad = 0;
            for (int64_t i = lo; i < hi; i++) {
                const float x = rgb_host[i];
                float y = x * 255.0f + 0.5f;
                y = y >= 0.0f ? y : 0.0f;
                const int k = y < 255.5f ? (int)y : 255;
                uint32_t a, b;
                memcpy(&a, &x, 4);
                memcpy(&b, &lut[k], 4);
                bad |= a ^ b;
                u8_host[i] = (uint8_t)k;
            }
            if (bad) { exact.store(0, std::memory_order_relaxed); return; }
        }
    };
    std::vector<std::thread> pool;
    for (int t = 1; t < nt; t++) pool.emplace_back(work);
    work();
    for (auto &th : pool) th.join();
    return exact.load();
}

extern "C" uint64_t aej_deflate_workspace_bytes(aej_ctx *ctx, int batch, int H, int W)
{
    QtGeom q;
    if (deflate_geometry(ctx, batch, H, W, q)) return 0;
    return deflate_workspace_bytes(batch, q.coeff_cap);
}

static int deflate_check(aej_ctx *ctx, const char *who, const void *a, const void *b, const void *ws, uint64_t ws_bytes, int batch, const QtGeom &q)
{
    if (call_in_flight(ctx)) return fail(ctx, AEJ_ERR_STATE, "%s between aej_encode_batch_begin and aej_encode_batch_end", who);
    if (!a || !b || !ws) return fail(ctx, AEJ_ERR_ARG, "NULL buffer");
    if (ws_bytes < deflate_workspace_bytes(batch, q.coeff_cap)) return fail(ctx, AEJ_ERR_CAPACITY, "workspace too small");
    return 0;
}

static int deflate_finish(aej_ctx *ctx, void *workspace, uint64_t stream_stride)
{
    AEJ_HIP_CHECK(hipGetLastError());
    AEJ_HIP_CHECK(hipMemcpyAsync(ctx->h_flag, workspace, sizeof(int), hipMemcpyDeviceToHost, ctx->stream));
    AEJ_HIP_CHECK(hipStreamSynchronize(ctx->stream));
    if (*ctx->h_flag == 2) return fail(ctx, AEJ_ERR_ARG, "counts: a layer's coefficient count is negative or exceeds the capacity the plan gives it (corrupt or stale counts buffer)");
    if (*ctx->h_flag) return fail(ctx, AEJ_ERR_CAPACITY, "a deflate stream does not fit stream_stride = %llu bytes (aej_deflate_stream_bound gives a safe size)", (unsigned long long)stream_stride);
    return 0;
}

extern "C" int aej_deflate_histogram(aej_ctx *ctx, const int32_t *coeffs, const int64_t *counts, int batch, int H, int W, int32_t *hist, void *workspace,
                                     uint64_t workspace_bytes)
{
    QtGeom q;
    int rc = deflate_geometry(ctx, batch, H, W, q);
    if (rc) return rc;
    if (!hist) return fail(ctx, AEJ_ERR_ARG, "NULL buffer");
    if ((rc = deflate_check(ctx, __func__, coeffs, counts, workspace, workspace_bytes, batch, q))) return rc;
    AEJ_HIP_CHECK(hipSetDevice(ctx->device));
    launch_deflate_parse(ctx->stream, coeffs, reinterpret_cast<const long long *>(counts), batch, q.coeff_stride, q.coeff_off, q.coeff_cap, hist, workspace);
    return deflate_finish(ctx, workspace, 0);
}

extern "C" int aej_deflate_batch(aej_ctx *ctx, const int32_t *coeffs, const int64_t *counts, int batch, int H, int W, const uint32_t *tables, int reuse_parse,
                                 uint8_t *streams, uint64_t stream_stride, int64_t *sizes, void *workspace, uint64_t workspace_bytes)
{
    QtGeom q;
    int rc = deflate_geometry(ctx, batch, H, W, q);
    if (rc) return rc;
    if (!streams || !sizes) return fail(ctx, AEJ_ERR_ARG, "NULL buffer");
    if ((rc = deflate_check(ctx, __func__, coeffs, counts, workspace, workspace_bytes, batch, q))) return rc;
    if (stream_stride < 16 || (stream_stride & 3)) return fail(ctx, AEJ_ERR_CAPACITY, "stream_stride must be a multiple of 4 and at least 16");
    if ((reinterpret_cast<uintptr_t>(streams) & 3) != 0) return fail(ctx, AEJ_ERR_ARG, "streams must be 4-byte aligned");
    AEJ_HIP_CHECK(hipSetDevice(ctx->device));
    launch_deflate(ctx->stream, coeffs, reinterpret_cast<const long long *>(counts), batch, q.coeff_stride, q.coeff_off, q.coeff_cap, tables, reuse_parse ? 1 : 0,
                   streams, stream_stride, reinterpret_cast<long long *>(sizes), workspace);
    return deflate_finish(ctx, workspace, stream_stride);
}

struct MetricsWs {
    double *part;
    MetricParts parts;
    unsigned char *ga, *gb;
    float *xa, *xb;
    float *pyr[2][4];
    int f, hp, wp;
    int lh[5], lw[5], lp[5];
    unsigned long long bytes;
};

static void carve_metrics(void *base, int B, int H, int W, MetricsWs &w)
{
    unsigned long long off = 0;
    auto take = [&](unsigned long long n) { void *p = base ? (char *)base + off : nullptr; off += (unsigned long long)align_up((long long)n, 256); return p; };
    w.ga = (unsigned char *)take((unsigned long long)B * H * W);
    w.gb = (unsigned char *)take((unsigned long long)B * H * W);
    w.f = (int)nearbyint((double)(H < W ? H : W) / 256.0);
    if (w.f < 1) w.f = 1;
    w.hp = H / w.f; w.wp = W / w.f;
    w.xa = (float *)take((unsigned long long)B * w.hp * w.wp * 4);
    w.xb = (float *)take((unsigned long long)B * w.hp * w.wp * 4);
    w.lh[0] = H; w.lw[0] = W; w.lp[0] = 0;
    for (int l = 1; l < 5; l++) {
        const int p = (w.lh[l - 1] % 2) > (w.lw[l - 1] % 2) ? (w.lh[l - 1] % 2) : (w.lw[l - 1] % 2);
        w.lp[l] = p;
        w.lh[l] = (w.lh[l - 1] + p) / 2;
        w.lw[l] = (w.lw[l - 1] + p) / 2;
        for (int i = 0; i < 2; i++) w.pyr[i][l - 1] = (float *)take((unsigned long long)B * 3 * w.lh[l] * w.lw[l] * 4);
    }
    MetricParts &P = w.parts;
    P.psnr_n = metric_prep_blocks((long long)H * W);
    P.grey_off = P.psnr_n;
    P.grey_n = ssim_partials(w.hp, w.wp);
    long long n = P.grey_off + P.grey_n;
    for (int l = 0; l < 5; l++) { P.lvl_off[l] = n; P.lvl_n[l] = ssim_partials(w.lh[l], w.lw[l]); n += 3 * P.lvl_n[l]; }
    P.stride = n;
    w.part = (double *)take((unsigned long long)B * n * sizeof(double));
    w.bytes = off;
}

extern "C" uint64_t aej_metrics_workspace_bytes(int batch, int H, int W)
{
    if (batch < 1 || H < 1 || W < 1) return 0;
    MetricsWs w;
    carve_metrics(nullptr, batch, H, W, w);
    return w.bytes;
}

extern "C" int aej_metrics_batch(aej_ctx *ctx, const float *img_a, const float *img_b, int batch, int H, int W, int which, double *out,
                                 void *workspace, uint64_t workspace_bytes)
{
    if (!ctx) return AEJ_ERR_ARG;
    if (call_in_flight(ctx)) return fail(ctx, AEJ_ERR_STATE, "%s between aej_encode_batch_begin and aej_encode_batch_end", __func__);
    if (!img_a || !img_b || !out || !workspace) return fail(ctx, AEJ_ERR_ARG, "NULL buffer");
    if (batch < 1 || H < 1 || W < 1) return fail(ctx, AEJ_ERR_ARG, "bad shape %d x %d x %d", batch, H, W);
    if ((which & ~7) || !(which & 7)) return fail(ctx, AEJ_ERR_ARG, "which must be a combination of AEJ_METRIC_PSNR | AEJ_METRIC_SSIM | AEJ_METRIC_MS_SSIM");
    AEJ_HIP_CHECK(hipSetDevice(ctx->device));
    MetricsWs w;
    carve_metrics(workspace, batch, H, W, w);
    if (w.bytes > workspace_bytes) return fail(ctx, AEJ_ERR_CAPACITY, "workspace too small: need %llu bytes, got %llu", w.bytes, (unsigned long long)workspace_bytes);
    const bool want_ssim = which & AEJ_METRIC_SSIM, want_ms = which & AEJ_METRIC_MS_SSIM;
    if (want_ssim && (w.hp < 11 || w.wp < 11)) return fail(ctx, AEJ_ERR_ARG, "Kernel size can't be greater than actual input size. Input size: %dx%d. Kernel size: 11x11", w.hp, w.wp);
    if (want_ms && (H < 161 || W < 161)) return fail(ctx, AEJ_ERR_ARG, "Invalid size of the input images, expected at least 161x161.");
    hipStream_t st = ctx->stream;
    float g11[11];
    {
        double e[11], sum = 0.0;
        for (int i = 0; i < 11; i++) { double c = (double)i - 5.0; e[i] = exp(-(c * c) / (2.0 * 1.5 * 1.5)); sum += e[i]; }
        for (int i = 0; i < 11; i++) g11[i] = (float)(e[i] / sum);
    }
    launch_metric_prep(st, img_a, img_b, batch, (long long)H * W, w.part, w.parts.stride, want_ssim ? w.ga : nullptr, want_ssim ? w.gb : nullptr);
    long long n_ssim = 0, n_level[5] = { 0, 0, 0, 0, 0 };
    if (want_ssim) {
        launch_metric_pool_grey(st, w.ga, w.gb, batch, H, W, w.f, w.hp, w.wp, w.xa, w.xb);
        launch_ssim_level(st, false, w.xa, w.xb, batch, 1, w.hp, w.wp, g11, w.part, w.parts.stride, w.parts.grey_off, true);
        n_ssim = (long long)(w.hp - 10) * (w.wp - 10);
    }
    if (want_ms) {
        for (int l = 0; l < 5; l++) {
            const float *xa = l == 0 ? img_a : w.pyr[0][l - 1], *xb = l == 0 ? img_b : w.pyr[1][l - 1];
            if (l > 0) {
                const float *pa = l == 1 ? img_a : w.pyr[0][l - 2], *pb = l == 1 ? img_b : w.pyr[1][l - 2];
                if (l == 1) {
                    if (w.lp[1] != 0) launch_pool2_rgb(st, pa, pb, batch, w.lh[0], w.lw[0], w.lp[1], w.lh[1], w.lw[1], w.pyr[0][0], w.pyr[1][0]);
                } else {
                    launch_pool2(st, false, pa, batch, 3, w.lh[l - 1], w.lw[l - 1], w.lp[l], w.lh[l], w.lw[l], w.pyr[0][l - 1]);
                    launch_pool2(st, false, pb, batch, 3, w.lh[l - 1], w.lw[l - 1], w.lp[l], w.lh[l], w.lw[l], w.pyr[1][l - 1]);
                }
            }
            const bool fused_pool = l == 0 && w.lp[1] == 0;
            launch_ssim_level(st, l == 0, xa, xb, batch, 3, w.lh[l], w.lw[l], g11, w.part, w.parts.stride, w.parts.lvl_off[l], l == 4,
                              fused_pool ? w.pyr[0][0] : nullptr, fused_pool ? w.pyr[1][0] : nullptr);
            n_level[l] = (long long)(w.lh[l] - 10) * (w.lw[l] - 10);
        }
    }
    launch_metric_final(st, w.part, w.parts, batch, (long long)H * W, n_ssim, n_level, out);
    AEJ_HIP_CHECK(hipGetLastError());
    return 0;
}

extern "C" int aej_get_hysteresis_stats(aej_ctx *ctx, int64_t *out_host)
{
    if (!ctx || !out_host) return AEJ_ERR_ARG;
    out_host[0] = ctx->n_encode_calls;
    out_host[1] = ctx->last_hyst_queued;
    return 0;
}

extern "C" int aej_set_graph_mode(aej_ctx *ctx, int mode)
{
    if (!ctx || mode < 0 || mode > 2) return AEJ_ERR_ARG;
    if (call_in_flight(ctx)) return fail(ctx, AEJ_ERR_STATE, "%s between aej_encode_batch_begin and aej_encode_batch_end", __func__);
    ctx->graph_mode = mode;
    if (mode == 0) drop_graphs(ctx);
    return 0;
}

extern "C" int aej_set_sub_batches(aej_ctx *ctx, int n)
{
    if (!ctx || n < 0 || n > aej_ctx::kMaxSub) return AEJ_ERR_ARG;
    ctx->sub_mode = n;
    return 0;
}

extern "C" int64_t aej_get_split_calls(aej_ctx *ctx) { return ctx ? (int64_t)ctx->n_split_calls : -1; }

extern "C" int aej_set_hw_queues(aej_ctx *ctx, int n)
{
    if (!ctx || n < 1) return AEJ_ERR_ARG;
    ctx->hw_queues = n;
    return 0;
}

extern "C" int aej_get_schedule_host(aej_ctx *ctx, int batch, int H, int W, int32_t *out_host)
{
    int rc = check_encode_args(ctx, batch, H, W);
    if (rc) return rc;
    if (!out_host) return fail(ctx, AEJ_ERR_ARG, "out_host is NULL");
    Geom g;
    if ((rc = make_geom(ctx, ctx->space, batch, H, W, g))) return rc;
    const int n = sub_batches(ctx, g, ctx->hw_queues), n_wide = sub_batches(ctx, g, 16);
    out_host[0] = ctx->hw_queues;
    out_host[1] = n;
    out_host[2] = (ctx->hw_queues < 8 && n_wide > n) ? 1 : 0;
    out_host[3] = 0;
    return 0;
}

namespace {
struct OptionDef { const char *name; int aej::Tuning::*field; int aej_ctx::*ctx_field; long long lo, hi; bool drops_graphs; };
const OptionDef kOptions[] = {
    { "color_strip", &aej::Tuning::color_strip, nullptr, 0, 1, true },
    { "color_strip_rows", &aej::Tuning::color_strip_rows, nullptr, 0, 64, true },
    { "color_workgroups", &aej::Tuning::color_workgroups, nullptr, 0, 1 << 16, true },
    { "planes_row_major", &aej::Tuning::planes_row_major, nullptr, 0, 1, true },
    { "dct64_kernel", &aej::Tuning::dct64_kernel, nullptr, 0, 4, true },
    { "dct_small_workgroups", &aej::Tuning::dct_small_workgroups, nullptr, 0, 1 << 16, true },
    { "sobel_lds", &aej::Tuning::sobel_lds, nullptr, 0, 1, true },
    { "sobel_xcd", &aej::Tuning::sobel_xcd, nullptr, 0, 1, true },
    { "dct_multi", &aej::Tuning::dct_multi, nullptr, 0, 1, true },
    { "sub_chain", nullptr, &aej_ctx::sub_chain, -1, 3, false },
    { "jpegdec_subseq_bits", nullptr, &aej_ctx::jd_subseq_bits, 32, 1 << 20, false },
};
const OptionDef *find_option(const char *name)
{
    if (!name) return nullptr;
    for (const OptionDef &o : kOptions) if (!strcmp(o.name, name)) return &o;
    return nullptr;
}
}

extern "C" int aej_set_option(aej_ctx *ctx, const char *name, int64_t value)
{
    if (!ctx) return AEJ_ERR_ARG;
    if (call_in_flight(ctx)) return fail(ctx, AEJ_ERR_STATE, "%s between aej_encode_batch_begin and aej_encode_batch_end", __func__);
    const OptionDef *o = find_option(name);
    if (!o) return fail(ctx, AEJ_ERR_ARG, "aej_set_option: unknown option '%s'", name ? name : "(null)");
    if (value < o->lo || value > o->hi || (o->field == &aej::Tuning::dct64_kernel && value != 0 && value != 1 && value != 4))
        return fail(ctx, AEJ_ERR_ARG, "aej_set_option: %s = %lld outside its range [%lld, %lld]", name, (long long)value, o->lo, o->hi);
    if (o->field) ctx->tune.*(o->field) = (int)value;
    else ctx->*(o->ctx_field) = (int)value;
    if (o->drops_graphs) drop_graphs(ctx);
    return 0;
}

extern "C" int aej_get_option(aej_ctx *ctx, const char *name, int64_t *value_host)
{
    if (!ctx || !value_host) return AEJ_ERR_ARG;
    const OptionDef *o = find_option(name);
    if (!o) return fail(ctx, AEJ_ERR_ARG, "aej_get_option: unknown option '%s'", name ? name : "(null)");
    *value_host = o->field ? ctx->tune.*(o->field) : ctx->*(o->ctx_field);
    return 0;
}

extern "C" int aej_test_fail_after_stage(aej_ctx *ctx, int stage)
{
    if (!ctx || stage < -1 || stage >= AEJ_N_STAGES) return AEJ_ERR_ARG;
    ctx->fail_after = stage;
    return 0;
}

extern "C" int aej_get_graph_stats(aej_ctx *ctx, int64_t *out_host)
{
    if (!ctx || !out_host) return AEJ_ERR_ARG;
    out_host[0] = (int64_t)ctx->n_graph_launches;
    out_host[1] = (int64_t)ctx->n_graph_captures;
    out_host[2] = (int64_t)ctx->graphs.size();
    return 0;
}

extern "C" int aej_set_stream(aej_ctx *ctx, void *hip_stream)
{
    if (!ctx) return AEJ_ERR_ARG;
    if (call_in_flight(ctx)) return fail(ctx, AEJ_ERR_STATE, "%s between aej_encode_batch_begin and aej_encode_batch_end", __func__);
    hipStream_t s = static_cast<hipStream_t>(hip_stream);
    if (s == ctx->stream) return 0;
    AEJ_HIP_CHECK(hipSetDevice(ctx->device));
    AEJ_HIP_CHECK(hipStreamSynchronize(ctx->stream));
    ctx->stream = s;
    return 0;
}

extern "C" int aej_set_profiling(aej_ctx *ctx, int enable)
{
    if (!ctx) return AEJ_ERR_ARG;
    if (call_in_flight(ctx)) return fail(ctx, AEJ_ERR_STATE, "%s between aej_encode_batch_begin and aej_encode_batch_end", __func__);
    ctx->profiling = enable != 0;
    return 0;
}

extern "C" int aej_get_stage_ms(aej_ctx *ctx, float *ms_host)
{
    if (!ctx || !ms_host) return AEJ_ERR_ARG;
    for (int i = 0; i < AEJ_N_STAGES; i++) ms_host[i] = ctx->stage_ms[i];
    return 0;
}

extern "C" const char *aej_stage_name(int i)
{
    static const char *names[AEJ_N_STAGES] = { "clear", "color_planes", "clahe_lut", "clahe_blur", "thresholds", "sobel_nms",
                                               "hysteresis", "quadtree", "dct2", "dct4", "dct8", "dct16", "dct32", "dct64", "dct128", "dct256", "dct512", "dct1024" };
    return i >= 0 && i < AEJ_N_STAGES ? names[i] : "";
}

struct LpipsWs {
    float *x, *y, *feats;
    double *partial;
    unsigned long long bytes;
};

static void carve_lpips(void *base, int B, const LpipsGeom &g, LpipsWs &w)
{
    unsigned long long off = 0;
    auto take = [&](unsigned long long n) { void *p = base ? (char *)base + off : nullptr; off += (unsigned long long)align_up((long long)n, 256); return p; };
    w.x = (float *)take((unsigned long long)B * g.x_elems * 4);
    w.y = (float *)take((unsigned long long)B * g.y_elems * 4);
    w.partial = (double *)take((unsigned long long)B * kLpipsTaps * g.max_blk * 8);
    w.bytes = off;
    w.feats = (float *)take((unsigned long long)B * g.feat_elems * 4);
}

extern "C" uint64_t aej_lpips_weights_bytes(void)
{
    long long off[kLpipsTaps][3];
    return (uint64_t)lpips_packed_floats(off) * 4;
}

extern "C" int64_t aej_lpips_param_count(void) { return lpips_param_floats(); }

extern "C" int aej_lpips_pack_weights_host(const float *params, int64_t n_params, void *packed_host)
{
    if (!params || !packed_host) return AEJ_ERR_ARG;
    if (n_params != lpips_param_floats()) return AEJ_ERR_ARG;
    lpips_pack_host(params, (float *)packed_host);
    return 0;
}

extern "C" uint64_t aej_lpips_features_bytes(int batch, int H, int W)
{
    LpipsGeom g;
    if (batch < 1 || !lpips_geom(H, W, g)) return 0;
    return (uint64_t)batch * g.feat_elems * 4;
}

extern "C" uint64_t aej_lpips_workspace_bytes(int batch, int H, int W)
{
    LpipsGeom g;
    if (batch < 1 || !lpips_geom(H, W, g)) return 0;
    LpipsWs w;
    carve_lpips(nullptr, batch, g, w);
    return w.bytes;
}

static int lpips_args(aej_ctx *ctx, const char *fn, const void *weights, int batch, int H, int W, LpipsGeom &g)
{
    if (call_in_flight(ctx)) return fail(ctx, AEJ_ERR_STATE, "%s between aej_encode_batch_begin and aej_encode_batch_end", fn);
    if (!weights) return fail(ctx, AEJ_ERR_ARG, "%s: NULL weights", fn);
    if (batch < 1 || H < 1 || W < 1) return fail(ctx, AEJ_ERR_ARG, "%s: bad shape %d x %d x %d", fn, batch, H, W);
    if (!lpips_geom(H, W, g))
        return fail(ctx, AEJ_ERR_ARG, "%s: LPIPS needs images of at least 31x31 (got %dx%d): AlexNet's second maxpool would have no output", fn, H, W);
    return 0;
}

extern "C" int aej_lpips_features(aej_ctx *ctx, const void *weights, const float *img, int batch, int H, int W, float *feats, void *workspace,
                                  uint64_t workspace_bytes)
{
    if (!ctx) return AEJ_ERR_ARG;
    LpipsGeom g;
    int rc = lpips_args(ctx, __func__, weights, batch, H, W, g);
    if (rc) return rc;
    if (!img || !feats || !workspace) return fail(ctx, AEJ_ERR_ARG, "NULL buffer");
    LpipsWs w;
    carve_lpips(workspace, batch, g, w);
    if (w.bytes > workspace_bytes) return fail(ctx, AEJ_ERR_CAPACITY, "workspace too small: need %llu bytes, got %llu", w.bytes, (unsigned long long)workspace_bytes);
    AEJ_HIP_CHECK(hipSetDevice(ctx->device));
    launch_lpips(ctx->stream, (const float *)weights, img, batch, g, w.x, w.y, feats, nullptr, nullptr, nullptr);
    AEJ_HIP_CHECK(hipGetLastError());
    return 0;
}

extern "C" int aej_lpips_batch(aej_ctx *ctx, const void *weights, const float *img_a, const float *feats_a, const float *img_b, int batch, int H, int W,
                               double *out, void *workspace, uint64_t workspace_bytes)
{
    if (!ctx) return AEJ_ERR_ARG;
    LpipsGeom g;
    int rc = lpips_args(ctx, __func__, weights, batch, H, W, g);
    if (rc) return rc;
    if (!img_a == !feats_a) return fail(ctx, AEJ_ERR_ARG, "exactly one of img_a and feats_a must be given");
    if (!img_b || !out || !workspace) return fail(ctx, AEJ_ERR_ARG, "NULL buffer");
    LpipsWs w;
    carve_lpips(workspace, batch, g, w);
    if (img_a) w.bytes += (unsigned long long)batch * g.feat_elems * 4;
    if (w.bytes > workspace_bytes) return fail(ctx, AEJ_ERR_CAPACITY, "workspace too small: need %llu bytes, got %llu", w.bytes, (unsigned long long)workspace_bytes);
    AEJ_HIP_CHECK(hipSetDevice(ctx->device));
    const float *wpk = (const float *)weights;
    if (img_a) {
        launch_lpips(ctx->stream, wpk, img_a, batch, g, w.x, w.y, w.feats, nullptr, nullptr, nullptr);
        feats_a = w.feats;
    }
    launch_lpips(ctx->stream, wpk, img_b, batch, g, w.x, w.y, nullptr, feats_a, w.partial, out);
    AEJ_HIP_CHECK(hipGetLastError());
    return 0;
}

static int jfif_args(aej_ctx *ctx, const char *fn, int batch, int H, int W, int n_q, int ss, int opt, JfifGeom &g)
{
    if (ctx && call_in_flight(ctx)) return fail(ctx, AEJ_ERR_STATE, "%s between aej_encode_batch_begin and aej_encode_batch_end", fn);
    if (ss < 0 || ss > 2) return fail(ctx, AEJ_ERR_ARG, "%s: subsampling %d (0 = 4:4:4, 1 = 4:2:2, 2 = 4:2:0)", fn, ss);
    if (opt != 0 && opt != 1) return fail(ctx, AEJ_ERR_ARG, "%s: optimize %d (0 or 1)", fn, opt);
    if (!jfif_geom(batch, H, W, n_q, g, ss, opt))
        return fail(ctx, AEJ_ERR_ARG, "%s: bad shape %d x %d x %d with %d qualities (1 <= H, W <= 65535)", fn, batch, H, W, n_q);
    return 0;
}

extern "C" uint64_t aej_jfif_workspace_bytes_opt(int batch, int H, int W, int n_q, int subsampling, int optimize)
{
    JfifGeom g;
    if ((optimize != 0 && optimize != 1) || !jfif_geom(batch, H, W, n_q, g, subsampling, optimize)) return 0;
    JfifBufs w;
    return jfif_carve(nullptr, g, w);
}

extern "C" uint64_t aej_jfif_workspace_bytes(int batch, int H, int W, int n_q) { return aej_jfif_workspace_bytes_opt(batch, H, W, n_q, 2, 0); }

extern "C" int aej_jfif_headers_host_opt(int quality, int H, int W, int subsampling, uint8_t *out_host, int capacity)
{
    JfifGeom g;
    if (quality < 1 || quality > 100 || !jfif_geom(1, H, W, 1, g, subsampling, 0) || !out_host) return AEJ_ERR_ARG;
    JfifParams p;
    jfif_params_host(quality, H, W, p, subsampling);
    if (capacity < p.hdr_len) return AEJ_ERR_CAPACITY;
    memcpy(out_host, p.hdr, p.hdr_len);
    return p.hdr_len;
}

extern "C" int aej_jfif_headers_host(int quality, int H, int W, uint8_t *out_host, int capacity)
{
    return aej_jfif_headers_host_opt(quality, H, W, 2, out_host, capacity);
}

extern "C" int aej_jfif_huffman_host(const int64_t *counts_host, uint8_t *bits_host, uint8_t *huffval_host, int capacity)
{
    if (!counts_host || !bits_host || !huffval_host || capacity < 0) return AEJ_ERR_ARG;
    unsigned char bits[16], vals[256];
    const int n = jfif_huffman_host((const long long *)counts_host, bits, vals);
    if (n < 0) return AEJ_ERR_ARG;
    if (n > capacity) return AEJ_ERR_CAPACITY;
    memcpy(bits_host, bits, 16);
    memcpy(huffval_host, vals, n);
    return n;
}

extern "C" int aej_jfif_encode_batch_opt(aej_ctx *ctx, const uint8_t *rgb, int batch, int H, int W, int n_q, const int32_t *qualities_host,
                                         int subsampling, int optimize, uint8_t *out, uint64_t out_capacity, int64_t *offsets, int64_t *lengths,
                                         uint64_t *total_host, void *workspace, uint64_t workspace_bytes)
{
    if (!ctx) return AEJ_ERR_ARG;
    JfifGeom g;
    int rc = jfif_args(ctx, __func__, batch, H, W, n_q, subsampling, optimize, g);
    if (rc) return rc;
    if (!rgb || !qualities_host || !offsets || !lengths || !total_host || !workspace) return fail(ctx, AEJ_ERR_ARG, "%s: NULL buffer", __func__);
    std::vector<JfifParams> par(n_q);
    for (int i = 0; i < n_q; i++) {
        if (qualities_host[i] < 1 || qualities_host[i] > 100) return fail(ctx, AEJ_ERR_ARG, "%s: quality %d outside 1..100", __func__, qualities_host[i]);
        jfif_params_host(qualities_host[i], H, W, par[i], subsampling);
    }
    JfifBufs w;
    const unsigned long long need = jfif_carve(workspace, g, w);
    if (need > workspace_bytes) return fail(ctx, AEJ_ERR_CAPACITY, "workspace too small: need %llu bytes, got %llu", need, (unsigned long long)workspace_bytes);
    AEJ_HIP_CHECK(hipSetDevice(ctx->device));
    AEJ_HIP_CHECK(launch_jfif_encode(ctx->stream, g, w, par.data(), rgb, out, out_capacity, (long long *)lengths, (long long *)offsets));
    long long total = 0;
    AEJ_HIP_CHECK(hipMemcpyAsync(&total, w.total, 8, hipMemcpyDeviceToHost, ctx->stream));
    AEJ_HIP_CHECK(hipStreamSynchronize(ctx->stream));
    *total_host = (uint64_t)total;
    if (out && (uint64_t)total > out_capacity)
        return fail(ctx, AEJ_ERR_CAPACITY, "%s: the files need %lld bytes, the output holds %llu (nothing was written)", __func__, total,
                    (unsigned long long)out_capacity);
    return 0;
}

extern "C" int aej_jfif_encode_batch(aej_ctx *ctx, const uint8_t *rgb, int batch, int H, int W, int n_q, const int32_t *qualities_host, uint8_t *out,
                                     uint64_t out_capacity, int64_t *offsets, int64_t *lengths, uint64_t *total_host, void *workspace,
                                     uint64_t workspace_bytes)
{
    return aej_jfif_encode_batch_opt(ctx, rgb, batch, H, W, n_q, qualities_host, 2, 0, out, out_capacity, offsets, lengths, total_host, workspace,
                                     workspace_bytes);
}

extern "C" int aej_jfif_recon_batch_opt(aej_ctx *ctx, int batch, int H, int W, int n_q, int subsampling, int optimize, uint8_t *rgb_out,
                                        void *workspace, uint64_t workspace_bytes)
{
    if (!ctx) return AEJ_ERR_ARG;
    JfifGeom g;
    int rc = jfif_args(ctx, __func__, batch, H, W, n_q, subsampling, optimize, g);
    if (rc) return rc;
    if (!rgb_out || !workspace) return fail(ctx, AEJ_ERR_ARG, "%s: NULL buffer", __func__);
    JfifBufs w;
    const unsigned long long need = jfif_carve(workspace, g, w);
    if (need > workspace_bytes) return fail(ctx, AEJ_ERR_CAPACITY, "workspace too small: need %llu bytes, got %llu", need, (unsigned long long)workspace_bytes);
    AEJ_HIP_CHECK(hipSetDevice(ctx->device));
    AEJ_HIP_CHECK(launch_jfif_recon(ctx->stream, g, w, rgb_out));
    return 0;
}

extern "C" int aej_jfif_recon_batch(aej_ctx *ctx, int batch, int H, int W, int n_q, uint8_t *rgb_out, void *workspace, uint64_t workspace_bytes)
{
    return aej_jfif_recon_batch_opt(ctx, batch, H, W, n_q, 2, 0, rgb_out, workspace, workspace_bytes);
}

extern "C" int aej_jpegdec_parse_host(const uint8_t *data_host, uint64_t nbytes, aej_jpegdec_desc *desc_host, char *msg, int msg_capacity)
{
    if (!desc_host) return AEJ_ERR_ARG;
    std::string m;
    const int rc = jpegdec_parse(data_host, nbytes, *desc_host, m);
    if (msg && msg_capacity > 0) {
        const size_t k = std::min(m.size(), (size_t)msg_capacity - 1);
        memcpy(msg, m.data(), k);
        msg[k] = 0;
    }
    return rc;
}

static bool jpegdec_descs_ok(const aej_jpegdec_desc *d, int n)
{
    if (!d || n < 1) return false;
    for (int i = 0; i < n; i++) {
        const aej_jpegdec_desc &e = d[i];
        const bool color = e.ncomp == 3 && ((e.hs == 1 && e.vs == 1) || (e.hs == 2 && (e.vs == 1 || e.vs == 2)));
        if (!(color || (e.ncomp == 1 && e.hs == 1 && e.vs == 1))) return false;
        if (e.width < 1 || e.height < 1 || e.width > 65535 || e.height > 65535 || e.scan_length < 0) return false;
        if (e.mcux != (e.width + 8 * e.hs - 1) / (8 * e.hs) || e.mcuy != (e.height + 8 * e.vs - 1) / (8 * e.vs)) return false;
        if (e.blocks_per_mcu != (e.ncomp == 1 ? 1 : e.hs * e.vs + 2) || e.restart_interval < 0) return false;
        const long long mcus = (long long)e.mcux * e.mcuy;
        if (e.n_segments != (e.restart_interval ? (mcus + e.restart_interval - 1) / e.restart_interval : 1)) return false;
    }
    return true;
}

extern "C" uint64_t aej_jpegdec_workspace_bytes(aej_ctx *ctx, const aej_jpegdec_desc *descs_host, int n)
{
    if (!ctx || !jpegdec_descs_ok(descs_host, n)) return 0;
    std::vector<JdFile> files;
    JdBufSizes z;
    jpegdec_layout(descs_host, n, ctx->jd_subseq_bits, files, z);
    JdBufs w;
    return jpegdec_carve(nullptr, n, z, w);
}

extern "C" int aej_jpegdec_batch(aej_ctx *ctx, const aej_jpegdec_desc *descs_host, int n, const uint8_t *scans, uint64_t scans_bytes,
                                 const int64_t *scan_offsets_host, uint8_t *out, uint64_t out_bytes, const int64_t *out_offsets_host,
                                 int32_t *status, void *workspace, uint64_t workspace_bytes)
{
    if (!ctx) return AEJ_ERR_ARG;
// ... 139 lines not shown
```

### adaptive_edge_aware_jpeg_amd/csrc/quadtree.hip

```cpp
#include "aej_common.h"
#include "aej_launch.h"

namespace aej {

__device__ __forceinline__ unsigned compact1by1(unsigned v)
{
    v &= 0x55555555u;
    v = (v | (v >> 1)) & 0x33333333u;
    v = (v | (v >> 2)) & 0x0F0F0F0Fu;
    v = (v | (v >> 4)) & 0x00FF00FFu;
    v = (v | (v >> 8)) & 0x0000FFFFu;
    return v;
}
__device__ __forceinline__ void morton_decode(unsigned m, int &x, int &y) { x = (int)compact1by1(m); y = (int)compact1by1(m >> 1); }

__device__ __forceinline__ long long lvl_off(int ncell, int lv)
{
    long long o = 0;
    for (int j = 0; j < lv; j++) { long long s = ncell >> j; o += s * s; }
    return o;
}

struct ChunkEdges {
    unsigned e0;
    bool e1, e2, e3, e4;
};

__device__ __forceinline__ ChunkEdges chunk_edges(const Geom &g, const QtGeom &q, int l, int b, const unsigned long long *__restrict__ edge_bits,
                                                  unsigned chunk, int lane)
{
    const int ncell = q.ncell[l], cell = q.cell;
    const int w = g.w[l], h = g.h[l], wpr = g.wpr[l];
    int ccx, ccy, lx, ly;
    morton_decode(chunk, ccx, ccy);
    morton_decode((unsigned)lane, lx, ly);
    const unsigned long long *src = edge_bits + (long long)b * g.bpstride + g.bpoff[l];
    ChunkEdges E;
    E.e0 = 0;
    if (cell == 4 && ncell >= 16) {
        const int X0 = ccx * 64, Y0 = ccy * 64;
        if (X0 < w && Y0 < h) {
            const unsigned long long *tile = src + bp_index(Y0, X0 >> 6, wpr);
            unsigned rows[8];
#pragma unroll
            for (int r = 0; r < 8; r++) {
                const int y = Y0 + 8 * ly + r;
                rows[r] = y < h ? (unsigned)((tile[8 * ly + r] >> (8 * lx)) & 0xFFull) : 0u;
            }
            const unsigned top = rows[0] | rows[1] | rows[2] | rows[3], bot = rows[4] | rows[5] | rows[6] | rows[7];
            E.e0 = ((top & 0x0Fu) ? 1u : 0u) | ((top & 0xF0u) ? 2u : 0u) | ((bot & 0x0Fu) ? 4u : 0u) | ((bot & 0xF0u) ? 8u : 0u);
        }
    } else {
#pragma unroll
        for (int i = 0; i < 4; i++) {
            const int cx = ccx * 16 + lx * 2 + (i & 1), cy = ccy * 16 + ly * 2 + (i >> 1);
            if (cx < ncell && cy < ncell && cx * cell < w && cy * cell < h) {
                int x0 = cx * cell, y0 = cy * cell;
                int x1 = min(x0 + cell, w), y1 = min(y0 + cell, h);
                bool e = false;
                for (int y = y0; y < y1; y++)
                    for (int xw = x0 >> 6; xw <= (x1 - 1) >> 6; xw++) {
                        int lo = max(x0, xw * 64) - xw * 64, hi = min(x1, xw * 64 + 64) - xw * 64;
                        unsigned long long mask = (hi - lo == 64) ? ~0ull : (((1ull << (hi - lo)) - 1ull) << lo);
                        e |= (src[bp_index(y, xw, wpr)] & mask) != 0;
                    }
                E.e0 |= (e ? 1u : 0u) << i;
            }
        }
    }
    E.e1 = E.e0 != 0;
    const unsigned long long m = __ballot(E.e1);
    E.e2 = ((m >> (lane & ~3)) & 0xFull) != 0;
    E.e3 = ((m >> (lane & ~15)) & 0xFFFFull) != 0;
    E.e4 = m != 0;
    return E;
}

__device__ __forceinline__ bool locate_chunk_block(const QtGeom &q, int nl, int bx, int &l, unsigned &chunk0)
{
    for (l = 0; l < nl; l++) {
        const int nb = (q.nchunk[l] + 3) >> 2;
        if (bx < nb) { chunk0 = (unsigned)bx * 4u; return true; }
        bx -= nb;
    }
    return false;
}

__global__ __launch_bounds__(256) void k_qt_upper(Geom g, QtGeom q, const unsigned long long *__restrict__ edge_bits, unsigned char *__restrict__ pyr_all)
{
    const int b = blockIdx.y;
    int l;
    unsigned chunk;
    if (!locate_chunk_block(q, g.nl, (int)blockIdx.x, l, chunk)) return;
    const int lane = threadIdx.x & 63;
    chunk += threadIdx.x >> 6;
    const int ncell = q.ncell[l], ltot = q.ltot[l], cell = q.cell;
    if ((long long)chunk >= q.nchunk[l] || ltot <= 4) return;
    int ccx, ccy;
    morton_decode(chunk, ccx, ccy);
    if (ccx * 16 * cell >= g.w[l] || ccy * 16 * cell >= g.h[l]) return;
    ChunkEdges E = chunk_edges(g, q, l, b, edge_bits, chunk, lane);
    if (lane == 0 && E.e4) {
        unsigned char *pyr = pyr_all + (long long)b * q.pyr_stride + q.pyr_off[l];
        for (int k = 5; k <= ltot && (cell << k) <= q.bmax; k++) {
            int side = ncell >> k;
            pyr[lvl_off(ncell, k) + (long long)((ccy * 16) >> k) * side + ((ccx * 16) >> k)] = 1;
        }
    }
}

struct CellNodes {
    int nsym;
    unsigned syms;
    int leaf_lvl;
};

__device__ __forceinline__ bool node_edge(const QtGeom &q, int l, const ChunkEdges &E, const unsigned char *__restrict__ pyr, int i, int cx, int cy, int lvn)
{
    switch (lvn) {
    case 0: return (E.e0 >> i) & 1u;
    case 1: return E.e1;
    case 2: return E.e2;
    case 3: return E.e3;
    case 4: return E.e4;
    default: {
        const int ncell = q.ncell[l], side = ncell >> lvn;
        return pyr[lvl_off(ncell, lvn) + (long long)(cy >> lvn) * side + (cx >> lvn)] != 0;
    }
    }
}

__device__ __forceinline__ CellNodes eval_cell(const QtGeom &q, int l, int w, int h, const ChunkEdges &E, const unsigned char *__restrict__ pyr, unsigned gidx,
                                               int cx, int cy)
{
    CellNodes r;
    r.nsym = 0; r.syms = 0; r.leaf_lvl = -1;
    const int ltot = q.ltot[l], cell = q.cell, i = (int)(gidx & 3u);
    int a = gidx == 0 ? ltot : min((int)(__ffs((int)gidx) - 1) >> 1, ltot);
    if (a < ltot) {
        int mask = ~((2 << a) - 1);
        int pcx = cx & mask, pcy = cy & mask;
        if (pcx * cell >= w || pcy * cell >= h) return r;
        int psize = cell << (a + 1);
        bool psplit = psize > q.bmax;
        if (!psplit && psize > q.bmin) psplit = node_edge(q, l, E, pyr, i, cx, cy, a + 1);
        if (!psplit) return r;
    }
    if (cx * cell >= w || cy * cell >= h) {
        r.nsym = 1; r.syms = 2u;
        return r;
    }
    for (int lvn = a; lvn >= 0; lvn--) {
        int size = cell << lvn;
        bool split = size > q.bmax;
        if (!split && size > q.bmin) split = node_edge(q, l, E, pyr, i, cx, cy, lvn);
        if (split) {
            r.syms |= 1u << (2 * r.nsym);
            r.nsym++;
        } else {
            r.nsym++;
            r.leaf_lvl = lvn;
            break;
        }
    }
    return r;
}

__device__ __forceinline__ void eval_lane(const QtGeom &q, int l, int w, int h, const ChunkEdges &E, const unsigned char *__restrict__ pyr, unsigned chunk,
                                          int lane, long long ncell2, CellNodes (&c)[4], int &cx0, int &cy0)
{
    int ccx, ccy, lx, ly;
    morton_decode(chunk, ccx, ccy);
    morton_decode((unsigned)lane, lx, ly);
    cx0 = ccx * 16 + lx * 2; cy0 = ccy * 16 + ly * 2;
    const unsigned g0 = chunk * 256u + (unsigned)lane * 4u;
#pragma unroll
    for (int i = 0; i < 4; i++) { c[i].nsym = 0; c[i].syms = 0; c[i].leaf_lvl = -1; }
    if ((long long)g0 >= ncell2) return;
    c[0] = eval_cell(q, l, w, h, E, pyr, g0, cx0, cy0);
    const int cell = q.cell;
    bool split1 = 2 * cell > q.bmax;
    if (!split1 && 2 * cell > q.bmin) split1 = E.e1;
    if (!(split1 && cx0 * cell < w && cy0 * cell < h)) return;
#pragma unroll
    for (int i = 1; i < 4; i++) {
        if ((long long)(g0 + i) >= ncell2) continue;
        const int cx = cx0 + (i & 1), cy = cy0 + (i >> 1);
        c[i].nsym = 1;
        if (cx * cell >= w || cy * cell >= h) c[i].syms = 2u;
        else if (cell > q.bmax || (cell > q.bmin && ((E.e0 >> i) & 1u))) c[i].syms = 1u;
        else c[i].leaf_lvl = 0;
    }
}

__device__ __forceinline__ unsigned pack_lane(const CellNodes (&c)[4])
{
    unsigned code = 0;
    if (c[0].nsym > 0) {
        if (c[0].nsym == 1 && c[0].syms == 2u) code = 3u;
        else {
            const int k = c[0].nsym - (c[0].leaf_lvl >= 0 ? 1 : 0);
            code = (c[0].leaf_lvl >= 0 ? 1u : 2u) | ((unsigned)k << 2);
        }
    }
#pragma unroll
    for (int i = 1; i < 4; i++) {
        const unsigned ci = c[i].nsym == 0 ? 0u : (c[i].syms == 2u ? 3u : c[i].syms == 1u ? 2u : 1u);
        code |= ci << (4 + 2 * i);
    }
    return code;
}

__device__ __forceinline__ void unpack_lane(unsigned code, unsigned g0, int ltot, CellNodes (&c)[4])
{
#pragma unroll
    for (int i = 0; i < 4; i++) { c[i].nsym = 0; c[i].syms = 0; c[i].leaf_lvl = -1; }
    const unsigned t = code & 3u;
    const int k = (int)((code >> 2) & 15u);
    if (t == 3u) { c[0].nsym = 1; c[0].syms = 2u; }
    else if (t != 0u) {
        const int a = g0 == 0 ? ltot : min((int)(__ffs((int)g0) - 1) >> 1, ltot);
        c[0].syms = 0x55555555u & ((1u << (2 * k)) - 1u);
        c[0].nsym = k + (t == 1u ? 1 : 0);
        if (t == 1u) c[0].leaf_lvl = a - k;
    }
#pragma unroll
    for (int i = 1; i < 4; i++) {
        const unsigned ci = (code >> (4 + 2 * i)) & 3u;
        if (ci) { c[i].nsym = 1; c[i].syms = ci == 3u ? 2u : ci == 2u ? 1u : 0u; c[i].leaf_lvl = ci == 1u ? 0 : -1; }
    }
}

__device__ __forceinline__ int wave_incl_scan(int v, int ) { return wave_scan_incl(v); }
__device__ __forceinline__ int wave_sum(int v) { return wave_total(v); }

__global__ __launch_bounds__(256) void k_qt_count(Geom g, QtGeom q, const unsigned long long *__restrict__ edge_bits,
                                                  const unsigned char *__restrict__ pyr_all, int *__restrict__ chunk_cnt,
                                                  unsigned short *__restrict__ lane_code)
{
    const int b = blockIdx.y;
    int l;
    unsigned chunk;
    if (!locate_chunk_block(q, g.nl, (int)blockIdx.x, l, chunk)) return;
    const int lane = threadIdx.x & 63;
    chunk += threadIdx.x >> 6;
    if ((long long)chunk >= q.nchunk[l]) return;
    const long long ncell2 = (long long)q.ncell[l] * q.ncell[l];
    const unsigned char *pyr = pyr_all + (long long)b * q.pyr_stride + q.pyr_off[l];
    {
        int ccx, ccy;
        morton_decode(chunk, ccx, ccy);
        if (ccx * 16 * q.cell >= g.w[l] || ccy * 16 * q.cell >= g.h[l]) {
            ChunkEdges Z;
            Z.e0 = 0; Z.e1 = Z.e2 = Z.e3 = Z.e4 = false;
            int ns = 0;
            if (lane == 0 && (long long)chunk * 256 < ncell2) ns = eval_cell(q, l, g.w[l], g.h[l], Z, pyr, chunk * 256u, ccx * 16, ccy * 16).nsym;
            lane_code[((long long)b * q.chunk_stride + q.chunk_off[l] + chunk) * 64 + lane] = (unsigned short)(ns ? 3u : 0u);
            if (lane == 0) {
                int *o = chunk_cnt + ((long long)b * q.chunk_stride + q.chunk_off[l] + chunk) * kChunkInts;
                o[0] = ns; o[1] = 0; o[2] = 0; o[3] = 0;
#pragma unroll
                for (int k = 0; k < kMaxSizes; k++) o[4 + k] = 0;
            }
            return;
        }
    }
    const ChunkEdges E = chunk_edges(g, q, l, b, edge_bits, chunk, lane);
    if (!E.e4 && (q.cell << 4) <= q.bmax) {
        CellNodes z[4];
#pragma unroll
        for (int i = 0; i < 4; i++) { z[i].nsym = 0; z[i].syms = 0; z[i].leaf_lvl = -1; }
        if (lane == 0 && (long long)chunk * 256 < ncell2) {
            int ccx, ccy;
            morton_decode(chunk, ccx, ccy);
            z[0] = eval_cell(q, l, g.w[l], g.h[l], E, pyr, chunk * 256u, ccx * 16, ccy * 16);
        }
        lane_code[((long long)b * q.chunk_stride + q.chunk_off[l] + chunk) * 64 + lane] = (unsigned short)pack_lane(z);
        if (lane == 0) {
            int *o = chunk_cnt + ((long long)b * q.chunk_stride + q.chunk_off[l] + chunk) * kChunkInts;
            const int lv = z[0].leaf_lvl, sz = lv >= 0 ? q.cell << lv : 0;
            o[0] = z[0].nsym; o[1] = lv >= 0 ? 1 : 0; o[2] = sz * sz; o[3] = 0;
#pragma unroll
            for (int k = 0; k < kMaxSizes; k++) o[4 + k] = (k == lv) ? 1 : 0;
        }
        return;
    }
    int nsym = 0, nleaf = 0, ncoef = 0;
    int nsz[kMaxSizes];
#pragma unroll
    for (int k = 0; k < kMaxSizes; k++) nsz[k] = 0;
    CellNodes cn[4];
    int cx0, cy0;
    eval_lane(q, l, g.w[l], g.h[l], E, pyr, chunk, lane, ncell2, cn, cx0, cy0);
    lane_code[((long long)b * q.chunk_stride + q.chunk_off[l] + chunk) * 64 + lane] = (unsigned short)pack_lane(cn);
#pragma unroll
    for (int i = 0; i < 4; i++) {
        const CellNodes &c = cn[i];
        nsym += c.nsym;
        if (c.leaf_lvl >= 0) {
            nleaf++;
            int s = q.cell << c.leaf_lvl;
            ncoef += s * s;
#pragma unroll
            for (int k = 0; k < kMaxSizes; k++) nsz[k] += (c.leaf_lvl == k) ? 1 : 0;
        }
    }
    static_assert(kMaxSizes <= 8, "three packed words hold the symbol count and 8 sizes");
    unsigned pk[3] = { (unsigned)nsym, 0u, 0u };
#pragma unroll
    for (int k = 0; k < kMaxSizes; k++) pk[(k + 1) / 3] |= (unsigned)nsz[k] << (10 * ((k + 1) % 3));
#pragma unroll
    for (int i = 0; i < 3; i++) pk[i] = (unsigned)wave_sum((int)pk[i]);
    nsym = (int)(pk[0] & 1023u);
    nleaf = 0; ncoef = 0;
#pragma unroll
    for (int k = 0; k < kMaxSizes; k++) {
        nsz[k] = k < q.nsizes ? (int)((pk[(k + 1) / 3] >> (10 * ((k + 1) % 3))) & 1023u) : 0;
        const int sz = q.cell << k;
        nleaf += nsz[k];
        ncoef += nsz[k] * sz * sz;
    }
    if (lane == 0) {
        int *o = chunk_cnt + ((long long)b * q.chunk_stride + q.chunk_off[l] + chunk) * kChunkInts;
        o[0] = nsym; o[1] = nleaf; o[2] = ncoef; o[3] = 0;
#pragma unroll
        for (int k = 0; k < kMaxSizes; k++) o[4 + k] = nsz[k];
    }
}

template <int kScanThreads>
__global__ __launch_bounds__(kScanThreads) void k_qt_scan(Geom g, QtGeom q, int *__restrict__ chunk_cnt, long long *__restrict__ counts,
                                                  int *__restrict__ work_count)
{
    constexpr int NQ = 3 + kMaxSizes;
    __shared__ int s_w[NQ][kScanThreads / 64];
    __shared__ int carry[NQ];
    const int tid = threadIdx.x, l = blockIdx.x, b = blockIdx.y;
    const int lane = tid & 63, wv = tid >> 6;
    int *base = chunk_cnt + ((long long)b * q.chunk_stride + q.chunk_off[l]) * kChunkInts;
    const int n = q.nchunk[l];
    const int nq = 3 + q.nsizes;
    if (tid < NQ) carry[tid] = 0;
    __syncthreads();
    static_assert(kChunkInts == 12 && NQ == 11, "a chunk record is three int4: (nsym, nleaf, ncoef, pad), leaves per size 0..3, 4..7");
    int4 *rec = reinterpret_cast<int4 *>(base);
    for (int start = 0; start < n; start += kScanThreads) {
        const int i = start + tid;
        int4 r0 = make_int4(0, 0, 0, 0), r1 = r0, r2 = r0;
        if (i < n) { r0 = rec[3 * i]; r1 = rec[3 * i + 1]; r2 = rec[3 * i + 2]; }
        int v[NQ] = { r0.x, r0.y, r0.z, r1.x, r1.y, r1.z, r1.w, r2.x, r2.y, r2.z, r2.w }, inc[NQ];
#pragma unroll
        for (int c = 0; c < NQ; c++) {
            if (c >= nq) v[c] = 0;
            inc[c] = wave_incl_scan(v[c], lane);
            if (lane == 63) s_w[c][wv] = inc[c];
        }
        __syncthreads();
        int o[NQ];
#pragma unroll
        for (int c = 0; c < NQ; c++) {
            int p = carry[c];
            for (int k = 0; k < wv; k++) p += s_w[c][k];
            o[c] = p + inc[c] - v[c];
        }
        if (i < n) {
            rec[3 * i] = make_int4(o[0], o[1], o[2], r0.w);
            rec[3 * i + 1] = make_int4(o[3], o[4], o[5], o[6]);
            rec[3 * i + 2] = make_int4(o[7], o[8], o[9], o[10]);
        }
        __syncthreads();
        if (tid < NQ) {
            int t = 0;
            for (int k = 0; k < kScanThreads / 64; k++) t += s_w[tid][k];
            carry[tid] += t;
        }
        __syncthreads();
    }
    if (tid == 0) {
        long long *o = counts + ((long long)b * 3 + l) * 4;
        o[0] = carry[2];
        o[1] = carry[1];
        o[2] = carry[0];
        o[3] = q.root[l];
    }
    if (work_count && tid < kMaxSizes) work_count[((long long)b * 3 + l) * kMaxSizes + tid] = tid < q.nsizes ? carry[3 + tid] : 0;
}

__global__ __launch_bounds__(256) void k_qt_emit(Geom g, QtGeom q, QtBuffers qb)
{
    const int b = blockIdx.y;
    int l;
    unsigned chunk;
    if (!locate_chunk_block(q, g.nl, (int)blockIdx.x, l, chunk)) return;
    const int lane = threadIdx.x & 63;
    chunk += threadIdx.x >> 6;
    if ((long long)chunk >= q.nchunk[l]) return;
    const int *coff = qb.chunk_cnt + ((long long)b * q.chunk_stride + q.chunk_off[l] + chunk) * kChunkInts;
    CellNodes c[4];
    const unsigned code = qb.lane_code[((long long)b * q.chunk_stride + q.chunk_off[l] + chunk) * 64 + lane];
    const unsigned long long originators = __ballot(code != 0);
    if (originators == 0) return;
    unpack_lane(code, chunk * 256u + (unsigned)lane * 4u, q.ltot[l], c);
    int ccx, ccy, lx, ly;
    morton_decode(chunk, ccx, ccy);
    morton_decode((unsigned)lane, lx, ly);
    const int cx0 = ccx * 16 + lx * 2, cy0 = ccy * 16 + ly * 2;
    int nsym = 0, nleaf = 0, ncoef = 0, n0 = 0;
#pragma unroll
    for (int i = 0; i < 4; i++) {
        nsym += c[i].nsym;
        if (c[i].leaf_lvl >= 0) { nleaf++; int s = q.cell << c[i].leaf_lvl; ncoef += s * s; }
        if (c[i].leaf_lvl == 0) n0++;
    }
    int sym_pos = coff[0], leaf_pos = coff[1], rank0 = 0, coef_pos = coff[2], rank_big = 0;
    if (originators != 1ull) {
        const int pk = nsym | nleaf << 10 | n0 << 20;
        const int pks = wave_incl_scan(pk, lane) - pk;
        sym_pos += pks & 1023;
        leaf_pos += (pks >> 10) & 1023;
        rank0 = (pks >> 20) & 1023;
        coef_pos += wave_incl_scan(ncoef, lane) - ncoef;
        const int big = c[0].leaf_lvl;
        for (int k = 1; k < q.nsizes; k++) {
            unsigned long long m = __ballot(big == k);
            if (big == k) rank_big = __popcll(m & ((1ull << lane) - 1ull));
        }
    }

    unsigned char *st = qb.states + (long long)b * q.state_stride + q.state_off[l];
    int *leaves = qb.leaves + ((long long)b * q.leaf_stride + q.leaf_off[l]) * 4;
#pragma unroll
    for (int i = 0; i < 4; i++) {
        for (int k = 0; k < c[i].nsym; k++) {
            if (sym_pos + k < q.state_cap[l]) st[sym_pos + k] = (unsigned char)((c[i].syms >> (2 * k)) & 3u);
            else *qb.overflow = 1;
        }
        sym_pos += c[i].nsym;
        if (c[i].leaf_lvl >= 0) {
            const int cx = cx0 + (i & 1), cy = cy0 + (i >> 1);
            const int size = q.cell << c[i].leaf_lvl;
            if (leaf_pos < q.leaf_cap[l] && (long long)coef_pos + (long long)size * size <= q.coeff_cap[l]) {
                reinterpret_cast<int4 *>(leaves)[leaf_pos] = make_int4(cx * q.cell, cy * q.cell, size, coef_pos);
                if (qb.work_count) {
                    const int k = c[i].leaf_lvl;
                    long long pos = (long long)coff[4 + k] + (k == 0 ? rank0 : rank_big);
                    long long seg = (long long)b * q.work_stride[k] + q.work_off[l][k];
                    if (seg + pos < qb.work_cap[k])
                        qb.work[k][seg + pos] = pack_work(cx * q.cell, cy * q.cell, coef_pos);
                    else
                        *qb.overflow = 1;
                    if (k == 0) rank0++;
                }
            } else {
                *qb.overflow = 1;
            }
            leaf_pos++;
            coef_pos += size * size;
        }
    }
}

static int chunk_blocks(const Geom &g, const QtGeom &q)
{
    int n = 0;
    for (int l = 0; l < g.nl; l++) n += (q.nchunk[l] + 3) / 4;
    return n;
}

void launch_qt_cells(hipStream_t st, const Geom &g, const QtGeom &q, const unsigned long long *edge_bits, const QtBuffers &qb)
{
    bool need = false;
    for (int l = 0; l < g.nl; l++) if (q.ltot[l] > 4 && (q.cell << 5) <= q.bmax) need = true;
    if (need) hipLaunchKernelGGL(k_qt_upper, dim3(chunk_blocks(g, q), g.B), dim3(256), 0, st, g, q, edge_bits, qb.pyr);
}
void launch_qt_count(hipStream_t st, const Geom &g, const QtGeom &q, const QtBuffers &qb)
{
    hipLaunchKernelGGL(k_qt_count, dim3(chunk_blocks(g, q), g.B), dim3(256), 0, st, g, q, qb.edge_bits, qb.pyr, qb.chunk_cnt, qb.lane_code);
}
void launch_qt_scan(hipStream_t st, const Geom &g, const QtGeom &q, const QtBuffers &qb)
{
    if (g.B <= 4) hipLaunchKernelGGL(k_qt_scan<1024>, dim3(g.nl, g.B), dim3(1024), 0, st, g, q, qb.chunk_cnt, qb.counts, qb.work_count);
    else hipLaunchKernelGGL(k_qt_scan<256>, dim3(g.nl, g.B), dim3(256), 0, st, g, q, qb.chunk_cnt, qb.counts, qb.work_count);
}
void launch_qt_emit(hipStream_t st, const Geom &g, const QtGeom &q, const QtBuffers &qb)
{
    hipLaunchKernelGGL(k_qt_emit, dim3(chunk_blocks(g, q), g.B), dim3(256), 0, st, g, q, qb);
}

}
```

### include/aej_testing.h

```cpp
#ifndef AEJ_TESTING_H
#define AEJ_TESTING_H

#include "aej.h"

#ifdef __cplusplus
extern "C" {
#endif

AEJ_API int aej_test_fail_after_stage(aej_ctx *ctx, int stage);

AEJ_API int aej_test_jpegprog_coefs(aej_ctx *ctx, const aej_jpegprog_frame *frames_host, const aej_jpegprog_scan *scans_host, int n,
                                    const uint8_t *data, uint64_t data_bytes, const int64_t *data_offsets_host, int n_levels,
                                    int16_t *coef_out, uint64_t coef_blocks, int32_t *status, void *workspace, uint64_t workspace_bytes);
AEJ_API int aej_test_jpegprog_coefs_host(const aej_jpegprog_frame *frame_host, const aej_jpegprog_scan *scans_host, const uint8_t *file_host,
                                         uint64_t nbytes, int n_levels, int16_t *coef_out_host, uint64_t coef_blocks);

#ifdef __cplusplus
}
#endif
#endif
```

Measured before the change: 84480 MP/s.

## Group quadtree chunks to fuse count, scan and upper-level evaluation

Adds a grouped quadtree path that processes runs of G Morton-ordered chunks per block. The group kernel evaluates the cells, keeps upper pyramid levels in registers, and writes per-group aggregates. A grouped emit kernel then prefix-sums the preceding aggregates and emits leaves, replacing the separate count, scan and emit launches, and often the upper-pyramid kernel and part of the memset too. The goal is to cut kernel launches and global pyramid traffic. In exchange, each emit block performs a redundant linear prefix over earlier groups and adds more complex index math.

```diff
diff --git a/adaptive_edge_aware_jpeg_amd/_lib.py b/adaptive_edge_aware_jpeg_amd/_lib.py
--- a/adaptive_edge_aware_jpeg_amd/_lib.py
+++ b/adaptive_edge_aware_jpeg_amd/_lib.py
@@ -203,6 +203,8 @@
     "aej_jpegprog_batch": (_I, [_P, _P, _P, _I, _P, _U64, _P, _P, _U64, _P, _P, _P, _U64]),
     "aej_test_jpegprog_coefs": (_I, [_P, _P, _P, _I, _P, _U64, _P, _I, _P, _U64, _P, _P, _U64]),
     "aej_test_jpegprog_coefs_host": (_I, [_P, _P, _P, _U64, _I, _P, _U64]),
+    "aej_test_qt_last": (_I, [_P, _P]),
+    "aej_test_qt_group_locate": (_I, [_I, _P, _P, _I, _I, _I, _I, _I, _P]),
 }
 
 INFLATE_STATUS = ["ok", "bad zlib header", "bad block type", "bad code lengths", "invalid literal/length or distance code",
diff --git a/adaptive_edge_aware_jpeg_amd/csrc/aej_common.h b/adaptive_edge_aware_jpeg_amd/csrc/aej_common.h
--- a/adaptive_edge_aware_jpeg_amd/csrc/aej_common.h
+++ b/adaptive_edge_aware_jpeg_amd/csrc/aej_common.h
@@ -53,9 +53,50 @@
     int sobel_lds = 0;
     int dct_multi = 1;
     int sobel_xcd = 1;
+    int qt_path = 0;
+    int qt_group = 0;
 };
 
 constexpr int kChunkInts = 4 + kMaxSizes;
+
+struct QtGroups {
+    int G[3];
+    int top[3];
+    int side[3];
+    int gw[3], gh[3];
+    int first[4];
+    int agg_stride;
+};
+__host__ __device__ inline unsigned qt_nth_in_plane(int side, int gw, int gh, int j)
+{
+    if (j >= gw * gh) return (unsigned)side * (unsigned)side;
+    int x0 = 0, y0 = 0;
+    unsigned m = 0;
+    for (int half = side >> 1; half >= 1; half >>= 1) {
+        for (int qd = 0; qd < 4; qd++) {
+            const int qx = x0 + (qd & 1) * half, qy = y0 + (qd >> 1) * half;
+            int cw = gw - qx, ch = gh - qy;
+            cw = cw < 0 ? 0 : cw > half ? half : cw;
+            ch = ch < 0 ? 0 : ch > half ? half : ch;
+            const int c = cw * ch;
+            if (j < c || qd == 3) { x0 = qx; y0 = qy; m = m * 4u + (unsigned)qd; break; }
+            j -= c;
+        }
+    }
+    return m;
+}
+__host__ __device__ inline bool qt_group_locate(const QtGroups &qg, int nl, int ticket, int &l, int &j, unsigned &m, unsigned &m_next)
+{
+    for (l = 0; l < nl; l++) {
+        if (ticket < qg.first[l + 1]) {
+            j = ticket - qg.first[l];
+            m = qt_nth_in_plane(qg.side[l], qg.gw[l], qg.gh[l], j);
+            m_next = qt_nth_in_plane(qg.side[l], qg.gw[l], qg.gh[l], j + 1);
+            return true;
+        }
+    }
+    return false;
+}
 constexpr int kMaxPlanes = 3072;
 
 constexpr int kMetricBand = 32;
diff --git a/adaptive_edge_aware_jpeg_amd/csrc/aej_launch.h b/adaptive_edge_aware_jpeg_amd/csrc/aej_launch.h
--- a/adaptive_edge_aware_jpeg_amd/csrc/aej_launch.h
+++ b/adaptive_edge_aware_jpeg_amd/csrc/aej_launch.h
@@ -53,6 +53,7 @@
     unsigned char *pyr;
     const unsigned long long *edge_bits;
     int *chunk_cnt;
+    int *grp_agg;
     unsigned short *lane_code;
     int *leaves;
     unsigned char *states;
@@ -67,6 +68,12 @@
 void launch_qt_count(hipStream_t st, const Geom &g, const QtGeom &q, const QtBuffers &qb);
 void launch_qt_scan(hipStream_t st, const Geom &g, const QtGeom &q, const QtBuffers &qb);
 void launch_qt_emit(hipStream_t st, const Geom &g, const QtGeom &q, const QtBuffers &qb);
+long long qt_group_records(const Geom &g, const QtGeom &q);
+bool qt_groups_plan(const Geom &g, const QtGeom &q, int G, QtGroups &qg);
+bool qt_need_upper(const Geom &g, const QtGeom &q, const QtGroups *qg );
+void launch_qt_upper(hipStream_t st, const Geom &g, const QtGeom &q, const unsigned long long *edge_bits, const QtBuffers &qb);
+void launch_qt_group(hipStream_t st, const Geom &g, const QtGeom &q, const QtGroups &qg, const QtBuffers &qb);
+void launch_qt_emit_group(hipStream_t st, const Geom &g, const QtGeom &q, const QtGroups &qg, const QtBuffers &qb);
 
 constexpr int kBigBlocks = 128;
 constexpr int kMaxBlock = 1024;
diff --git a/adaptive_edge_aware_jpeg_amd/csrc/api.hip b/adaptive_edge_aware_jpeg_amd/csrc/api.hip
--- a/adaptive_edge_aware_jpeg_amd/csrc/api.hip
+++ b/adaptive_edge_aware_jpeg_amd/csrc/api.hip
@@ -51,6 +51,7 @@
     unsigned long long graph_clock = 0, n_graph_launches = 0, n_graph_captures = 0;
     int sub_mode = 0;
     int hw_queues = 4;
+    int qt_last[4] = { 0, 0, 0, 0 };
     int fail_after = -1;
     static constexpr int kMaxSub = 8;
     int dct_crowded = 0;
@@ -321,6 +322,7 @@
     w.zero_end = c.base ? c.base + c.off : nullptr;
     w.qb.chunk_cnt = c.take<int>((long long)g.B * q.chunk_stride * kChunkInts);
     w.qb.lane_code = c.take<unsigned short>((long long)g.B * q.chunk_stride * 64);
+    w.qb.grp_agg = c.take<int>((long long)g.B * qt_group_records(g, q) * kChunkInts);
     if (with_work) {
         w.qb.work_count = c.take<int>((long long)g.B * 3 * kMaxSizes);
         for (int k = 0; k < q.nsizes; k++) {
@@ -559,13 +561,23 @@
 static int run_quadtree(aej_ctx *ctx, const Geom &g, const QtGeom &q, QtWs &w, const unsigned long long *edge_bits)
 {
     hipStream_t st = ctx->stream;
-    if (ctx->capturing) launch_zero(st, w.zero_begin, (size_t)(w.zero_end - w.zero_begin));
-    else AEJ_HIP_CHECK(hipMemsetAsync(w.zero_begin, 0, (size_t)(w.zero_end - w.zero_begin), st));
+    QtGroups qg;
+    const bool grouped = ctx->tune.qt_path != 3 && qt_groups_plan(g, q, ctx->tune.qt_group, qg);
+    const bool upper = qt_need_upper(g, q, grouped ? &qg : nullptr);
+    char *zero_begin = (upper || !grouped) ? w.zero_begin : reinterpret_cast<char *>(w.qb.overflow);
+    if (ctx->capturing) launch_zero(st, zero_begin, (size_t)(w.zero_end - zero_begin));
+    else AEJ_HIP_CHECK(hipMemsetAsync(zero_begin, 0, (size_t)(w.zero_end - zero_begin), st));
     w.qb.edge_bits = edge_bits;
-    launch_qt_cells(st, g, q, edge_bits, w.qb);
-    launch_qt_count(st, g, q, w.qb);
-    launch_qt_scan(st, g, q, w.qb);
-    launch_qt_emit(st, g, q, w.qb);
+    if (upper) launch_qt_upper(st, g, q, edge_bits, w.qb);
+    if (grouped) {
+        launch_qt_group(st, g, q, qg, w.qb);
+        launch_qt_emit_group(st, g, q, qg, w.qb);
+    } else {
+        launch_qt_count(st, g, q, w.qb);
+        launch_qt_scan(st, g, q, w.qb);
+        launch_qt_emit(st, g, q, w.qb);
+    }
+    ctx->qt_last[0] = grouped ? 2 : 3; ctx->qt_last[1] = grouped ? qg.G[0] : 0; ctx->qt_last[2] = upper ? 1 : 0; ctx->qt_last[3] = grouped ? qg.first[g.nl] : 0;
     AEJ_HIP_CHECK(hipGetLastError());
     return 0;
 }
@@ -1743,6 +1755,8 @@
     { "sobel_lds", &aej::Tuning::sobel_lds, nullptr, 0, 1, true },
     { "sobel_xcd", &aej::Tuning::sobel_xcd, nullptr, 0, 1, true },
     { "dct_multi", &aej::Tuning::dct_multi, nullptr, 0, 1, true },
+    { "qt_path", &aej::Tuning::qt_path, nullptr, 0, 3, true },
+    { "qt_group", &aej::Tuning::qt_group, nullptr, 0, 64, true },
     { "sub_chain", nullptr, &aej_ctx::sub_chain, -1, 3, false },
     { "jpegdec_subseq_bits", nullptr, &aej_ctx::jd_subseq_bits, 32, 1 << 20, false },
 };
@@ -1760,7 +1774,9 @@
     if (call_in_flight(ctx)) return fail(ctx, AEJ_ERR_STATE, "%s between aej_encode_batch_begin and aej_encode_batch_end", __func__);
     const OptionDef *o = find_option(name);
     if (!o) return fail(ctx, AEJ_ERR_ARG, "aej_set_option: unknown option '%s'", name ? name : "(null)");
-    if (value < o->lo || value > o->hi || (o->field == &aej::Tuning::dct64_kernel && value != 0 && value != 1 && value != 4))
+    if (value < o->lo || value > o->hi || (o->field == &aej::Tuning::dct64_kernel && value != 0 && value != 1 && value != 4) ||
+        (o->field == &aej::Tuning::qt_path && value == 1) ||
+        (o->field == &aej::Tuning::qt_group && value != 0 && value != 4 && value != 16 && value != 64))
         return fail(ctx, AEJ_ERR_ARG, "aej_set_option: %s = %lld outside its range [%lld, %lld]", name, (long long)value, o->lo, o->hi);
     if (o->field) ctx->tune.*(o->field) = (int)value;
     else ctx->*(o->ctx_field) = (int)value;
@@ -1774,6 +1790,37 @@
     const OptionDef *o = find_option(name);
     if (!o) return fail(ctx, AEJ_ERR_ARG, "aej_get_option: unknown option '%s'", name ? name : "(null)");
     *value_host = o->field ? ctx->tune.*(o->field) : ctx->*(o->ctx_field);
+    return 0;
+}
+
+extern "C" int aej_test_qt_last(aej_ctx *ctx, int32_t *out_host)
+{
+    if (!ctx || !out_host) return AEJ_ERR_ARG;
+    for (int i = 0; i < 4; i++) out_host[i] = ctx->qt_last[i];
+    return 0;
+}
+
+extern "C" int aej_test_qt_group_locate(int nl, const int32_t *h, const int32_t *w, int min_size, int max_size, int batch, int G, int ticket,
+                                        int32_t *out_host)
+{
+    if (nl < 1 || nl > 3 || !h || !w || !out_host) return AEJ_ERR_ARG;
+    Geom g;
+    memset(&g, 0, sizeof g);
+    g.B = batch; g.nl = nl;
+    for (int l = 0; l < nl; l++) { g.h[l] = h[l]; g.w[l] = w[l]; }
+    QtGeom q;
+    int rc = make_qtgeom(nullptr, g, min_size, max_size, q, true);
+    if (rc) return rc;
+    QtGroups qg;
+    for (int i = 0; i < 8; i++) out_host[i] = 0;
+    if (!qt_groups_plan(g, q, G, qg)) return 0;
+    out_host[0] = 1;
+    out_host[1] = qg.first[nl];
+    out_host[7] = qt_need_upper(g, q, &qg) ? 1 : 0;
+    int l, j;
+    unsigned m, m_next;
+    if (ticket < 0 || !qt_group_locate(qg, nl, ticket, l, j, m, m_next)) return 0;
+    out_host[2] = l; out_host[3] = qg.G[l]; out_host[4] = (int)(m * (unsigned)qg.G[l]); out_host[5] = (int)(m_next * (unsigned)qg.G[l]); out_host[6] = j;
     return 0;
 }
 
diff --git a/adaptive_edge_aware_jpeg_amd/csrc/quadtree.hip b/adaptive_edge_aware_jpeg_amd/csrc/quadtree.hip
--- a/adaptive_edge_aware_jpeg_amd/csrc/quadtree.hip
+++ b/adaptive_edge_aware_jpeg_amd/csrc/quadtree.hip
@@ -24,6 +24,8 @@
 struct ChunkEdges {
     unsigned e0;
     bool e1, e2, e3, e4;
+    int top;
+    unsigned up;
 };
 
 __device__ __forceinline__ ChunkEdges chunk_edges(const Geom &g, const QtGeom &q, int l, int b, const unsigned long long *__restrict__ edge_bits,
@@ -36,7 +38,7 @@
     morton_decode((unsigned)lane, lx, ly);
     const unsigned long long *src = edge_bits + (long long)b * g.bpstride + g.bpoff[l];
     ChunkEdges E;
-    E.e0 = 0;
+    E.e0 = 0; E.top = 4; E.up = 0;
     if (cell == 4 && ncell >= 16) {
         const int X0 = ccx * 64, Y0 = ccy * 64;
         if (X0 < w && Y0 < h) {
@@ -124,6 +126,7 @@
     case 3: return E.e3;
     case 4: return E.e4;
     default: {
+        if (lvn <= E.top) return (E.up >> (lvn - 5)) & 1u;
         const int ncell = q.ncell[l], side = ncell >> lvn;
         return pyr[lvl_off(ncell, lvn) + (long long)(cy >> lvn) * side + (cx >> lvn)] != 0;
     }
@@ -234,6 +237,64 @@
 __device__ __forceinline__ int wave_incl_scan(int v, int ) { return wave_scan_incl(v); }
 __device__ __forceinline__ int wave_sum(int v) { return wave_total(v); }
 
+__device__ __forceinline__ unsigned count_chunk(const Geom &g, const QtGeom &q, int l, const ChunkEdges &E, const unsigned char *__restrict__ pyr,
+                                                unsigned chunk, int lane, long long ncell2, bool outside, int (&cnt)[3 + kMaxSizes])
+{
+#pragma unroll
+    for (int c = 0; c < 3 + kMaxSizes; c++) cnt[c] = 0;
+    int ccx, ccy;
+    morton_decode(chunk, ccx, ccy);
+    if (outside) {
+        int ns = 0;
+        if (lane == 0 && (long long)chunk * 256 < ncell2) ns = eval_cell(q, l, g.w[l], g.h[l], E, pyr, chunk * 256u, ccx * 16, ccy * 16).nsym;
+        cnt[0] = __builtin_amdgcn_readfirstlane(ns);
+        return ns ? 3u : 0u;
+    }
+    if (!E.e4 && (q.cell << 4) <= q.bmax) {
+        CellNodes z[4];
+#pragma unroll
+        for (int i = 0; i < 4; i++) { z[i].nsym = 0; z[i].syms = 0; z[i].leaf_lvl = -1; }
+        if (lane == 0 && (long long)chunk * 256 < ncell2) z[0] = eval_cell(q, l, g.w[l], g.h[l], E, pyr, chunk * 256u, ccx * 16, ccy * 16);
+        const int lv = __builtin_amdgcn_readfirstlane(z[0].leaf_lvl), sz = lv >= 0 ? q.cell << lv : 0;
+        cnt[0] = __builtin_amdgcn_readfirstlane(z[0].nsym); cnt[1] = lv >= 0 ? 1 : 0; cnt[2] = sz * sz;
+#pragma unroll
+        for (int k = 0; k < kMaxSizes; k++) cnt[3 + k] = (k == lv) ? 1 : 0;
+        return pack_lane(z);
+    }
+    int nsym = 0;
+    int nsz[kMaxSizes];
+#pragma unroll
+    for (int k = 0; k < kMaxSizes; k++) nsz[k] = 0;
+    CellNodes cn[4];
+    int cx0, cy0;
+    eval_lane(q, l, g.w[l], g.h[l], E, pyr, chunk, lane, ncell2, cn, cx0, cy0);
+#pragma unroll
+    for (int i = 0; i < 4; i++) {
+        const CellNodes &c = cn[i];
+        nsym += c.nsym;
+        if (c.leaf_lvl >= 0) {
+#pragma unroll
+            for (int k = 0; k < kMaxSizes; k++) nsz[k] += (c.leaf_lvl == k) ? 1 : 0;
+        }
+    }
+    static_assert(kMaxSizes <= 8, "three packed words hold the symbol count and 8 sizes");
+    unsigned pk[3] = { (unsigned)nsym, 0u, 0u };
+#pragma unroll
+    for (int k = 0; k < kMaxSizes; k++) pk[(k + 1) / 3] |= (unsigned)nsz[k] << (10 * ((k + 1) % 3));
+#pragma unroll
+    for (int i = 0; i < 3; i++) pk[i] = (unsigned)wave_sum((int)pk[i]);
+    cnt[0] = (int)(pk[0] & 1023u);
+#pragma unroll
+    for (int k = 0; k < kMaxSizes; k++) {
+        const int n = k < q.nsizes ? (int)((pk[(k + 1) / 3] >> (10 * ((k + 1) % 3))) & 1023u) : 0;
+        const int sz = q.cell << k;
+        cnt[3 + k] = n;
+        cnt[1] += n;
+        cnt[2] += n * sz * sz;
+    }
+    return pack_lane(cn);
+}
+
 __global__ __launch_bounds__(256) void k_qt_count(Geom g, QtGeom q, const unsigned long long *__restrict__ edge_bits,
                                                   const unsigned char *__restrict__ pyr_all, int *__restrict__ chunk_cnt,
                                                   unsigned short *__restrict__ lane_code)
@@ -247,84 +308,20 @@
     if ((long long)chunk >= q.nchunk[l]) return;
     const long long ncell2 = (long long)q.ncell[l] * q.ncell[l];
     const unsigned char *pyr = pyr_all + (long long)b * q.pyr_stride + q.pyr_off[l];
-    {
-        int ccx, ccy;
-        morton_decode(chunk, ccx, ccy);
-        if (ccx * 16 * q.cell >= g.w[l] || ccy * 16 * q.cell >= g.h[l]) {
-            ChunkEdges Z;
-            Z.e0 = 0; Z.e1 = Z.e2 = Z.e3 = Z.e4 = false;
-            int ns = 0;
-            if (lane == 0 && (long long)chunk * 256 < ncell2) ns = eval_cell(q, l, g.w[l], g.h[l], Z, pyr, chunk * 256u, ccx * 16, ccy * 16).nsym;
-            lane_code[((long long)b * q.chunk_stride + q.chunk_off[l] + chunk) * 64 + lane] = (unsigned short)(ns ? 3u : 0u);
-            if (lane == 0) {
-                int *o = chunk_cnt + ((long long)b * q.chunk_stride + q.chunk_off[l] + chunk) * kChunkInts;
-                o[0] = ns; o[1] = 0; o[2] = 0; o[3] = 0;
-#pragma unroll
-                for (int k = 0; k < kMaxSizes; k++) o[4 + k] = 0;
-            }
-            return;
-        }
-    }
-    const ChunkEdges E = chunk_edges(g, q, l, b, edge_bits, chunk, lane);
-    if (!E.e4 && (q.cell << 4) <= q.bmax) {
-        CellNodes z[4];
-#pragma unroll
-        for (int i = 0; i < 4; i++) { z[i].nsym = 0; z[i].syms = 0; z[i].leaf_lvl = -1; }
-        if (lane == 0 && (long long)chunk * 256 < ncell2) {
-            int ccx, ccy;
-            morton_decode(chunk, ccx, ccy);
-            z[0] = eval_cell(q, l, g.w[l], g.h[l], E, pyr, chunk * 256u, ccx * 16, ccy * 16);
-        }
-        lane_code[((long long)b * q.chunk_stride + q.chunk_off[l] + chunk) * 64 + lane] = (unsigned short)pack_lane(z);
-        if (lane == 0) {
-            int *o = chunk_cnt + ((long long)b * q.chunk_stride + q.chunk_off[l] + chunk) * kChunkInts;
-            const int lv = z[0].leaf_lvl, sz = lv >= 0 ? q.cell << lv : 0;
-            o[0] = z[0].nsym; o[1] = lv >= 0 ? 1 : 0; o[2] = sz * sz; o[3] = 0;
-#pragma unroll
-            for (int k = 0; k < kMaxSizes; k++) o[4 + k] = (k == lv) ? 1 : 0;
-        }
-        return;
-    }
-    int nsym = 0, nleaf = 0, ncoef = 0;
-    int nsz[kMaxSizes];
-#pragma unroll
-    for (int k = 0; k < kMaxSizes; k++) nsz[k] = 0;
-    CellNodes cn[4];
-    int cx0, cy0;
-    eval_lane(q, l, g.w[l], g.h[l], E, pyr, chunk, lane, ncell2, cn, cx0, cy0);
-    lane_code[((long long)b * q.chunk_stride + q.chunk_off[l] + chunk) * 64 + lane] = (unsigned short)pack_lane(cn);
-#pragma unroll
-    for (int i = 0; i < 4; i++) {
-        const CellNodes &c = cn[i];
-        nsym += c.nsym;
-        if (c.leaf_lvl >= 0) {
-            nleaf++;
-            int s = q.cell << c.leaf_lvl;
-            ncoef += s * s;
-#pragma unroll
-            for (int k = 0; k < kMaxSizes; k++) nsz[k] += (c.leaf_lvl == k) ? 1 : 0;
-        }
-    }
-    static_assert(kMaxSizes <= 8, "three packed words hold the symbol count and 8 sizes");
-    unsigned pk[3] = { (unsigned)nsym, 0u, 0u };
-#pragma unroll
-    for (int k = 0; k < kMaxSizes; k++) pk[(k + 1) / 3] |= (unsigned)nsz[k] << (10 * ((k + 1) % 3));
-#pragma unroll
-    for (int i = 0; i < 3; i++) pk[i] = (unsigned)wave_sum((int)pk[i]);
-    nsym = (int)(pk[0] & 1023u);
-    nleaf = 0; ncoef = 0;
-#pragma unroll
-    for (int k = 0; k < kMaxSizes; k++) {
-        nsz[k] = k < q.nsizes ? (int)((pk[(k + 1) / 3] >> (10 * ((k + 1) % 3))) & 1023u) : 0;
-        const int sz = q.cell << k;
-        nleaf += nsz[k];
-        ncoef += nsz[k] * sz * sz;
-    }
+    int ccx, ccy;
+    morton_decode(chunk, ccx, ccy);
+    const bool outside = ccx * 16 * q.cell >= g.w[l] || ccy * 16 * q.cell >= g.h[l];
+    ChunkEdges E;
+    if (outside) { E.e0 = 0; E.e1 = E.e2 = E.e3 = E.e4 = false; E.top = 4; E.up = 0; }
+    else E = chunk_edges(g, q, l, b, edge_bits, chunk, lane);
+    int cnt[3 + kMaxSizes];
+    const unsigned code = count_chunk(g, q, l, E, pyr, chunk, lane, ncell2, outside, cnt);
+    lane_code[((long long)b * q.chunk_stride + q.chunk_off[l] + chunk) * 64 + lane] = (unsigned short)code;
     if (lane == 0) {
         int *o = chunk_cnt + ((long long)b * q.chunk_stride + q.chunk_off[l] + chunk) * kChunkInts;
-        o[0] = nsym; o[1] = nleaf; o[2] = ncoef; o[3] = 0;
-#pragma unroll
-        for (int k = 0; k < kMaxSizes; k++) o[4 + k] = nsz[k];
+        o[0] = cnt[0]; o[1] = cnt[1]; o[2] = cnt[2]; o[3] = 0;
+#pragma unroll
+        for (int k = 0; k < kMaxSizes; k++) o[4 + k] = cnt[3 + k];
     }
 }
 
@@ -386,18 +383,9 @@
     if (work_count && tid < kMaxSizes) work_count[((long long)b * 3 + l) * kMaxSizes + tid] = tid < q.nsizes ? carry[3 + tid] : 0;
 }
 
-__global__ __launch_bounds__(256) void k_qt_emit(Geom g, QtGeom q, QtBuffers qb)
-{
-    const int b = blockIdx.y;
-    int l;
-    unsigned chunk;
-    if (!locate_chunk_block(q, g.nl, (int)blockIdx.x, l, chunk)) return;
-    const int lane = threadIdx.x & 63;
-    chunk += threadIdx.x >> 6;
-    if ((long long)chunk >= q.nchunk[l]) return;
-    const int *coff = qb.chunk_cnt + ((long long)b * q.chunk_stride + q.chunk_off[l] + chunk) * kChunkInts;
+__device__ __forceinline__ void emit_chunk(const QtGeom &q, const QtBuffers &qb, int b, int l, unsigned chunk, int lane, unsigned code, const int *coff)
+{
     CellNodes c[4];
-    const unsigned code = qb.lane_code[((long long)b * q.chunk_stride + q.chunk_off[l] + chunk) * 64 + lane];
     const unsigned long long originators = __ballot(code != 0);
     if (originators == 0) return;
     unpack_lane(code, chunk * 256u + (unsigned)lane * 4u, q.ltot[l], c);
@@ -460,6 +448,250 @@
     }
 }
 
+__global__ __launch_bounds__(256) void k_qt_emit(Geom g, QtGeom q, QtBuffers qb)
+{
+    const int b = blockIdx.y;
+    int l;
+    unsigned chunk;
+    if (!locate_chunk_block(q, g.nl, (int)blockIdx.x, l, chunk)) return;
+    const int lane = threadIdx.x & 63;
+    chunk += threadIdx.x >> 6;
+    if ((long long)chunk >= q.nchunk[l]) return;
+    const int *coff = qb.chunk_cnt + ((long long)b * q.chunk_stride + q.chunk_off[l] + chunk) * kChunkInts;
+    const unsigned code = qb.lane_code[((long long)b * q.chunk_stride + q.chunk_off[l] + chunk) * 64 + lane];
+    emit_chunk(q, qb, b, l, chunk, lane, code, coff);
+}
+
+__device__ __forceinline__ void chunk_rows(const Geom &g, int l, const unsigned long long *__restrict__ src, unsigned chunk, int lx, int ly, unsigned (&rows)[8])
+{
+    int ccx, ccy;
+    morton_decode(chunk, ccx, ccy);
+    const int X0 = ccx * 64, Y0 = ccy * 64, h = g.h[l];
+#pragma unroll
+    for (int r = 0; r < 8; r++) rows[r] = 0u;
+    if (X0 < g.w[l] && Y0 < h) {
+        const unsigned char *t = reinterpret_cast<const unsigned char *>(src + bp_index(Y0, X0 >> 6, g.wpr[l])) + 64 * ly + lx;
+#pragma unroll
+        for (int r = 0; r < 8; r++)
+            if (Y0 + 8 * ly + r < h) rows[r] = t[8 * r];
+    }
+}
+__device__ __forceinline__ unsigned rows_e0(const unsigned (&rows)[8])
+{
+    const unsigned top = rows[0] | rows[1] | rows[2] | rows[3], bot = rows[4] | rows[5] | rows[6] | rows[7];
+    return ((top & 0x0Fu) ? 1u : 0u) | ((top & 0xF0u) ? 2u : 0u) | ((bot & 0x0Fu) ? 4u : 0u) | ((bot & 0xF0u) ? 8u : 0u);
+}
+__device__ __forceinline__ int tail_syms(const Geom &g, const QtGeom &q, int l, const unsigned char *__restrict__ pyr, unsigned gi, int G)
+{
+    ChunkEdges Z;
+    Z.e0 = 0; Z.e1 = Z.e2 = Z.e3 = Z.e4 = false; Z.top = 4; Z.up = 0;
+    const unsigned chunk = gi * (unsigned)G;
+    int ccx, ccy;
+    morton_decode(chunk, ccx, ccy);
+    return eval_cell(q, l, g.w[l], g.h[l], Z, pyr, chunk * 256u, ccx * 16, ccy * 16).nsym;
+}
+
+constexpr int kQtMaxGroup = 64;
+
+__global__ __launch_bounds__(256) void k_qt_group(Geom g, QtGeom q, QtGroups qg, const unsigned long long *__restrict__ edge_bits,
+                                                  const unsigned char *__restrict__ pyr_all, int *__restrict__ chunk_cnt,
+                                                  unsigned short *__restrict__ lane_code, int *__restrict__ grp_agg)
+{
+    constexpr int NQ = 3 + kMaxSizes;
+    __shared__ unsigned char s_any[kQtMaxGroup];
+    __shared__ int s_off[kQtMaxGroup][kChunkInts];
+    __shared__ int s_wtot[4][kChunkInts];
+    __shared__ int s_tail;
+    const int b = blockIdx.y, tid = threadIdx.x, lane = tid & 63, wv = tid >> 6;
+    int l, j;
+    unsigned m, m_next;
+    if (!qt_group_locate(qg, g.nl, (int)blockIdx.x, l, j, m, m_next)) return;
+    const int G = qg.G[l], cpw = G >= 4 ? G >> 2 : 1, nw = G / cpw;
+    const unsigned chunk0 = m * (unsigned)G;
+    const long long ncell2 = (long long)q.ncell[l] * q.ncell[l];
+    const unsigned char *pyr = pyr_all + (long long)b * q.pyr_stride + q.pyr_off[l];
+    const unsigned long long *src = edge_bits + (long long)b * g.bpstride + g.bpoff[l];
+    const long long rec0 = (long long)b * q.chunk_stride + q.chunk_off[l] + chunk0;
+    int lx, ly;
+    morton_decode((unsigned)lane, lx, ly);
+    if (tid < kQtMaxGroup && tid >= G) s_any[tid] = 0;
+    if (tid == 0) s_tail = 0;
+
+    unsigned long long e0pk = 0;
+    if (wv < nw) {
+        unsigned cur[8], nxt[8] = { 0u, 0u, 0u, 0u, 0u, 0u, 0u, 0u };
+        chunk_rows(g, l, src, chunk0 + (unsigned)(wv * cpw), lx, ly, cur);
+        for (int i = 0; i < cpw; i++) {
+            const int ci = wv * cpw + i;
+            if (i + 1 < cpw) chunk_rows(g, l, src, chunk0 + (unsigned)ci + 1u, lx, ly, nxt);
+            const unsigned e0 = rows_e0(cur);
+            e0pk |= (unsigned long long)e0 << (4 * i);
+            const bool any = __ballot(e0 != 0) != 0;
+            if (lane == 0) s_any[ci] = any ? 1 : 0;
+#pragma unroll
+            for (int r = 0; r < 8; r++) cur[r] = nxt[r];
+        }
+    }
+    __syncthreads();
+    const unsigned long long M = __ballot(s_any[lane] != 0);
+
+    int run[NQ];
+#pragma unroll
+    for (int c = 0; c < NQ; c++) run[c] = 0;
+    if (wv < nw) {
+        for (int i = 0; i < cpw; i++) {
+            const int ci = wv * cpw + i;
+            const unsigned chunk = chunk0 + (unsigned)ci;
+            ChunkEdges E;
+            E.e0 = (unsigned)(e0pk >> (4 * i)) & 15u;
+            E.e1 = E.e0 != 0;
+            const unsigned long long mm = __ballot(E.e1);
+            E.e2 = ((mm >> (lane & ~3)) & 0xFull) != 0;
+            E.e3 = ((mm >> (lane & ~15)) & 0xFFFFull) != 0;
+            E.e4 = mm != 0;
+            E.top = qg.top[l];
+            E.up = (((M >> (ci & ~3)) & 0xFull) ? 1u : 0u) | (((M >> (ci & ~15)) & 0xFFFFull) ? 2u : 0u) | (M ? 4u : 0u);
+            int ccx, ccy;
+            morton_decode(chunk, ccx, ccy);
+            const bool outside = ccx * 16 * q.cell >= g.w[l] || ccy * 16 * q.cell >= g.h[l];
+            int cnt[NQ];
+            const unsigned code = count_chunk(g, q, l, E, pyr, chunk, lane, ncell2, outside, cnt);
+            lane_code[(rec0 + ci) * 64 + lane] = (unsigned short)code;
+            if (lane == 0) {
+                s_off[ci][0] = run[0]; s_off[ci][1] = run[1]; s_off[ci][2] = run[2]; s_off[ci][3] = 0;
+#pragma unroll
+                for (int k = 0; k < kMaxSizes; k++) s_off[ci][4 + k] = run[3 + k];
+            }
+#pragma unroll
+            for (int c = 0; c < NQ; c++) run[c] += cnt[c];
+        }
+        if (lane == 0) {
+            s_wtot[wv][0] = run[0]; s_wtot[wv][1] = run[1]; s_wtot[wv][2] = run[2]; s_wtot[wv][3] = 0;
+#pragma unroll
+            for (int k = 0; k < kMaxSizes; k++) s_wtot[wv][4 + k] = run[3 + k];
+        }
+    }
+    int tl = 0;
+    for (unsigned base = m + 1u; base < m_next; base += 256u) {
+        const unsigned gi = base + (unsigned)tid;
+        if (gi < m_next) tl += tail_syms(g, q, l, pyr, gi, G);
+    }
+    if (m + 1u < m_next) {
+        tl = wave_total(tl);
+        if (lane == 0 && tl) atomicAdd(&s_tail, tl);
+    }
+    __syncthreads();
+
+    if (tid < G) {
+        int o[kChunkInts];
+#pragma unroll
+        for (int c = 0; c < kChunkInts; c++) o[c] = s_off[tid][c];
+        const int wq = tid / cpw;
+        for (int k = 0; k < wq; k++) {
+#pragma unroll
+            for (int c = 0; c < kChunkInts; c++) o[c] += s_wtot[k][c];
+        }
+        int4 *rec = reinterpret_cast<int4 *>(chunk_cnt + (rec0 + tid) * kChunkInts);
+        rec[0] = make_int4(o[0], o[1], o[2], 0);
+        rec[1] = make_int4(o[4], o[5], o[6], o[7]);
+        rec[2] = make_int4(o[8], o[9], o[10], o[11]);
+    }
+    if (tid == 64) {
+        int o[kChunkInts];
+#pragma unroll
+        for (int c = 0; c < kChunkInts; c++) o[c] = 0;
+        for (int k = 0; k < nw; k++) {
+#pragma unroll
+            for (int c = 0; c < kChunkInts; c++) o[c] += s_wtot[k][c];
+        }
+        const int t = s_tail;
+        int4 *rec = reinterpret_cast<int4 *>(grp_agg + (((long long)b * 3 + l) * qg.agg_stride + j) * kChunkInts);
+        rec[0] = make_int4(o[0] + t, o[1], o[2], t);
+        rec[1] = make_int4(o[4], o[5], o[6], o[7]);
+        rec[2] = make_int4(o[8], o[9], o[10], o[11]);
+    }
+}
+
+__global__ __launch_bounds__(256) void k_qt_emit_group(Geom g, QtGeom q, QtGroups qg, QtBuffers qb)
+{
+    __shared__ int s_w[4][kChunkInts];
+    __shared__ int s_off[kQtMaxGroup][kChunkInts];
+    const int b = blockIdx.y, tid = threadIdx.x, lane = tid & 63, wv = tid >> 6;
+    int l, j;
+    unsigned m, m_next;
+    if (!qt_group_locate(qg, g.nl, (int)blockIdx.x, l, j, m, m_next)) return;
+    const int G = qg.G[l], cpw = G >= 4 ? G >> 2 : 1, nw = G / cpw;
+    const unsigned chunk0 = m * (unsigned)G;
+    const long long rec0 = (long long)b * q.chunk_stride + q.chunk_off[l] + chunk0;
+    const int4 *agg = reinterpret_cast<const int4 *>(qb.grp_agg + (((long long)b * 3 + l) * qg.agg_stride) * kChunkInts);
+    static_assert(kChunkInts == 12, "a record is three int4: (nsym, nleaf, ncoef, pad), leaves per size 0..3, 4..7");
+    int acc[kChunkInts];
+#pragma unroll
+    for (int c = 0; c < kChunkInts; c++) acc[c] = 0;
+    for (int i = tid; i < j; i += 256) {
+        const int4 r0 = agg[3 * i], r1 = agg[3 * i + 1], r2 = agg[3 * i + 2];
+        acc[0] += r0.x; acc[1] += r0.y; acc[2] += r0.z;
+        acc[4] += r1.x; acc[5] += r1.y; acc[6] += r1.z; acc[7] += r1.w;
+        acc[8] += r2.x; acc[9] += r2.y; acc[10] += r2.z; acc[11] += r2.w;
+    }
+#pragma unroll
+    for (int c = 0; c < kChunkInts; c++) {
+        const int t = wave_total(acc[c]);
+        if (lane == 0) s_w[wv][c] = t;
+    }
+    __syncthreads();
+    int pre[kChunkInts];
+#pragma unroll
+    for (int c = 0; c < kChunkInts; c++) pre[c] = s_w[0][c] + s_w[1][c] + s_w[2][c] + s_w[3][c];
+    if (tid < G) {
+        const int4 *rec = reinterpret_cast<const int4 *>(qb.chunk_cnt + (rec0 + tid) * kChunkInts);
+        const int4 r0 = rec[0], r1 = rec[1], r2 = rec[2];
+        s_off[tid][0] = pre[0] + r0.x; s_off[tid][1] = pre[1] + r0.y; s_off[tid][2] = pre[2] + r0.z; s_off[tid][3] = 0;
+        s_off[tid][4] = pre[4] + r1.x; s_off[tid][5] = pre[5] + r1.y; s_off[tid][6] = pre[6] + r1.z; s_off[tid][7] = pre[7] + r1.w;
+        s_off[tid][8] = pre[8] + r2.x; s_off[tid][9] = pre[9] + r2.y; s_off[tid][10] = pre[10] + r2.z; s_off[tid][11] = pre[11] + r2.w;
+    }
+    __syncthreads();
+    if (wv < nw) {
+        unsigned code = qb.lane_code[(rec0 + wv * cpw) * 64 + lane];
+        for (int i = 0; i < cpw; i++) {
+            const int ci = wv * cpw + i;
+            unsigned next = 0;
+            if (i + 1 < cpw) next = qb.lane_code[(rec0 + ci + 1) * 64 + lane];
+            emit_chunk(q, qb, b, l, chunk0 + (unsigned)ci, lane, code, s_off[ci]);
+            code = next;
+        }
+    }
+    const int4 own = agg[3 * j];
+    if (wv == 0 && m + 1u < m_next) {
+        const unsigned char *pyr = qb.pyr + (long long)b * q.pyr_stride + q.pyr_off[l];
+        unsigned char *st = qb.states + (long long)b * q.state_stride + q.state_off[l];
+        int pos = pre[0] + own.x - own.w;
+        for (unsigned base = m + 1u; base < m_next; base += 64u) {
+            const unsigned gi = base + (unsigned)lane;
+            const int ns = gi < m_next ? tail_syms(g, q, l, pyr, gi, G) : 0;
+            const unsigned long long mk = __ballot(ns != 0);
+            if (ns) {
+                const int p = pos + __popcll(mk & ((1ull << lane) - 1ull));
+                if (p < q.state_cap[l]) st[p] = (unsigned char)2u;
+                else *qb.overflow = 1;
+            }
+            pos += __popcll(mk);
+        }
+    }
+    if (tid == 0 && m_next == (unsigned)qg.side[l] * (unsigned)qg.side[l]) {
+        const int4 o1 = agg[3 * j + 1], o2 = agg[3 * j + 2];
+        long long *o = qb.counts + ((long long)b * 3 + l) * 4;
+        o[0] = pre[2] + own.z;
+        o[1] = pre[1] + own.y;
+        o[2] = pre[0] + own.x;
+        o[3] = q.root[l];
+        if (qb.work_count) {
+            const int tot[kMaxSizes] = { pre[4] + o1.x, pre[5] + o1.y, pre[6] + o1.z, pre[7] + o1.w, pre[8] + o2.x, pre[9] + o2.y, pre[10] + o2.z, pre[11] + o2.w };
+#pragma unroll
+            for (int k = 0; k < kMaxSizes; k++) qb.work_count[((long long)b * 3 + l) * kMaxSizes + k] = k < q.nsizes ? tot[k] : 0;
+        }
+    }
+}
 static int chunk_blocks(const Geom &g, const QtGeom &q)
 {
     int n = 0;
@@ -467,11 +699,74 @@
     return n;
 }
 
+bool qt_need_upper(const Geom &g, const QtGeom &q, const QtGroups *qg)
+{
+    for (int l = 0; l < g.nl; l++) {
+        const int top = qg ? qg->top[l] : 4;
+        if (q.ltot[l] > top && ((long long)q.cell << (top + 1)) <= q.bmax) return true;
+    }
+    return false;
+}
+void launch_qt_upper(hipStream_t st, const Geom &g, const QtGeom &q, const unsigned long long *edge_bits, const QtBuffers &qb)
+{
+    hipLaunchKernelGGL(k_qt_upper, dim3(chunk_blocks(g, q), g.B), dim3(256), 0, st, g, q, edge_bits, qb.pyr);
+}
 void launch_qt_cells(hipStream_t st, const Geom &g, const QtGeom &q, const unsigned long long *edge_bits, const QtBuffers &qb)
 {
-    bool need = false;
-    for (int l = 0; l < g.nl; l++) if (q.ltot[l] > 4 && (q.cell << 5) <= q.bmax) need = true;
-    if (need) hipLaunchKernelGGL(k_qt_upper, dim3(chunk_blocks(g, q), g.B), dim3(256), 0, st, g, q, edge_bits, qb.pyr);
+    if (qt_need_upper(g, q, nullptr)) launch_qt_upper(st, g, q, edge_bits, qb);
+}
+
+static bool qt_groups_served(const Geom &g, const QtGeom &q)
+{
+    if (q.cell != 4) return false;
+    for (int l = 0; l < g.nl; l++) if (q.ncell[l] < 16) return false;
+    return true;
+}
+static int qt_groups_fill(const Geom &g, const QtGeom &q, int G, QtGroups &qg)
+{
+    int n = 0, stride = 1;
+    for (int l = 0; l < 3; l++) {
+        if (l >= g.nl) { qg.G[l] = 1; qg.top[l] = 4; qg.side[l] = 1; qg.gw[l] = qg.gh[l] = 0; qg.first[l + 1] = n; continue; }
+        const int Gl = G < q.nchunk[l] ? G : q.nchunk[l];
+        const int lg = ilog2(Gl) / 2, px = (16 * q.cell) << lg;
+        qg.G[l] = Gl;
+        qg.top[l] = 4 + lg;
+        qg.side[l] = 1 << ((ilog2(q.nchunk[l]) - 2 * lg) / 2);
+        qg.gw[l] = (g.w[l] + px - 1) / px < qg.side[l] ? (g.w[l] + px - 1) / px : qg.side[l];
+        qg.gh[l] = (g.h[l] + px - 1) / px < qg.side[l] ? (g.h[l] + px - 1) / px : qg.side[l];
+        qg.first[l] = n;
+        n += qg.gw[l] * qg.gh[l];
+        qg.first[l + 1] = n;
+        if (qg.gw[l] * qg.gh[l] > stride) stride = qg.gw[l] * qg.gh[l];
+    }
+    qg.agg_stride = stride;
+    return n;
+}
+long long qt_group_records(const Geom &g, const QtGeom &q)
+{
+    if (!qt_groups_served(g, q)) return 0;
+    QtGroups qg;
+    qt_groups_fill(g, q, 4, qg);
+    return 3LL * qg.agg_stride;
+}
+bool qt_groups_plan(const Geom &g, const QtGeom &q, int G, QtGroups &qg)
+{
+    qg = QtGroups{};
+    if (!qt_groups_served(g, q)) return false;
+    if (G != 4 && G != 16 && G != 64) {
+        for (G = kQtMaxGroup; G > 4; G /= 4)
+            if ((long long)qt_groups_fill(g, q, G, qg) * g.B >= 512) break;
+    }
+    qt_groups_fill(g, q, G, qg);
+    return true;
+}
+void launch_qt_group(hipStream_t st, const Geom &g, const QtGeom &q, const QtGroups &qg, const QtBuffers &qb)
+{
+    hipLaunchKernelGGL(k_qt_group, dim3(qg.first[g.nl], g.B), dim3(256), 0, st, g, q, qg, qb.edge_bits, qb.pyr, qb.chunk_cnt, qb.lane_code, qb.grp_agg);
+}
+void launch_qt_emit_group(hipStream_t st, const Geom &g, const QtGeom &q, const QtGroups &qg, const QtBuffers &qb)
+{
+    hipLaunchKernelGGL(k_qt_emit_group, dim3(qg.first[g.nl], g.B), dim3(256), 0, st, g, q, qg, qb);
 }
 void launch_qt_count(hipStream_t st, const Geom &g, const QtGeom &q, const QtBuffers &qb)
 {
diff --git a/include/aej_testing.h b/include/aej_testing.h
--- a/include/aej_testing.h
+++ b/include/aej_testing.h
@@ -9,6 +9,10 @@
 
 AEJ_API int aej_test_fail_after_stage(aej_ctx *ctx, int stage);
 
+AEJ_API int aej_test_qt_last(aej_ctx *ctx, int32_t *out_host);
+AEJ_API int aej_test_qt_group_locate(int nl, const int32_t *h, const int32_t *w, int min_size, int max_size, int batch, int G, int ticket,
+                                     int32_t *out_host);
+
 AEJ_API int aej_test_jpegprog_coefs(aej_ctx *ctx, const aej_jpegprog_frame *frames_host, const aej_jpegprog_scan *scans_host, int n,
                                     const uint8_t *data, uint64_t data_bytes, const int64_t *data_offsets_host, int n_levels,
                                     int16_t *coef_out, uint64_t coef_blocks, int32_t *status, void *workspace, uint64_t workspace_bytes);
```

After: 84410 MP/s, median of 2. About the same (-0.1%).
